# nktoan/h-edit

Measured on AMD Instinct MI355X. Metric: edited images/sec (512^2, 50 steps, K Langevin), higher is better.
Workload: dtype bf16

## Files before the change

### h-edit_amd/csrc/attn.hip

```cpp
#include "common.h"
#include "kernels.h"
#include <type_traits>

namespace {

typedef __attribute__((ext_vector_type(4))) unsigned u32x4;

__device__ __forceinline__ float fast_exp2(float x) { return __builtin_amdgcn_exp2f(x); }
#ifndef SA_BURST
#define SA_BURST 0
#endif

template <int D>
struct HeadCfg {
  static constexpr int DP = (D + 15) / 16 * 16;
  static constexpr int DK = DP / 16;
  static constexpr int DT = (D + 31) / 32;
  static constexpr int KS = DP + 8;
  static constexpr int DCH = D / 8;
};

__device__ __forceinline__ bf16x8 pack_p8(const float* p) {
  union { uint32_t u[4]; bf16x8 v; } x;
  x.u[0] = pack_bf16x2(p[0], p[1]);
// ... 547 lines not shown
    write_out(o[0], 1.0f / denom(0), q_base);
  }
}

template <int D, int QG, int NS>
int launch_self(const SelfAttnParams& p, hipStream_t st) {
  using C = SelfCfg<D, QG>;
#ifdef SA_OCC1
  constexpr int LDS = C::TOTAL > 84 * 1024 ? C::TOTAL : 84 * 1024;
#else
  constexpr int LDS = C::TOTAL;
#endif
  if (int rc = hedit_dyn_lds(reinterpret_cast<const void*>(&self_attn_kernel<D, QG, NS>), LDS)) return rc;
  dim3 grid(cdiv(p.N, 128 * QG) * p.heads * p.B);
  hipLaunchKernelGGL((self_attn_kernel<D, QG, NS>), grid, dim3(256), LDS, st, p);
  LAUNCH_CHECK();
  return HEDIT_OK;
}

constexpr int CTXP = HEDIT_CTXP;
constexpr int WS = 100;

template <int D>
struct CrossSmem {
  using H = HeadCfg<D>;
  static constexpr int K_BYTES = 96 * H::KS * 2;
  static constexpr int V_BYTES = H::DT * 32 * WS * 2;
  static constexpr int MIX_BYTES = 96 * WS * 2;
  static constexpr int BV_BYTES = 96 * 4;
  static constexpr int TOTAL = K_BYTES + V_BYTES + MIX_BYTES + BV_BYTES;
};

template <int D>
__global__ __launch_bounds__(256, (D <= 80 ? 2 : 1)) void cross_attn_kernel(CrossAttnParams p) {
  using H = HeadCfg<D>;
  using S = CrossSmem<D>;
  extern __shared__ __attribute__((aligned(16))) char smem[];
  bf16_t* sK = reinterpret_cast<bf16_t*>(smem);
  bf16_t* sV = reinterpret_cast<bf16_t*>(smem + S::K_BYTES);
  bf16_t* sM = reinterpret_cast<bf16_t*>(smem + S::K_BYTES + S::V_BYTES);
  float* sB = reinterpret_cast<float*>(smem + S::K_BYTES + S::V_BYTES + S::MIX_BYTES);

  const int tid = threadIdx.x, lane = tid & 63, wave = tid >> 6;
  const int ql = lane & 31, hi = lane >> 5;
  const int h = blockIdx.y;
  const int item = blockIdx.z;
  const bool is_pair = item < p.n_pairs;
  const int b0 = is_pair ? p.pair_src[item] : p.singles[item - p.n_pairs];
  const int b1 = is_pair ? p.pair_tar[item] : -1;
  const int q_row = blockIdx.x * 128 + wave * 32 + ql;
  const bool q_ok = q_row < p.N;

  for (int i = tid; i < (S::K_BYTES + S::V_BYTES) / 8; i += 256) reinterpret_cast<uint2*>(smem)[i] = make_uint2(0, 0);
  if (is_pair) {
    const bf16_t* src = p.mixT + (long)item * 96 * 96;
    for (int i = tid; i < 96 * 12; i += 256) {
      const int row = i / 12, c = i - row * 12;
      const uint4 u = *reinterpret_cast<const uint4*>(src + row * 96 + c * 8);
      uint2* dst = reinterpret_cast<uint2*>(sM + row * WS + c * 8);
      dst[0] = make_uint2(u.x, u.y);
      dst[1] = make_uint2(u.z, u.w);
    }
    if (tid < 96) sB[tid] = p.bvec[(long)item * 96 + tid];
  }
  __syncthreads();

  auto stage = [&](int b) {
    const bf16_t* kbase = p.k + (long)b * CTXP * p.ldk + h * D;
    for (int idx = tid; idx < CTXP * H::DCH; idx += 256) {
      const int row = idx / H::DCH, c = idx - row * H::DCH;
      *reinterpret_cast<uint4*>(sK + row * H::KS + c * 8) =
          *reinterpret_cast<const uint4*>(kbase + (long)row * p.ldk + c * 8);
    }
    const bf16_t* vbase = p.vt + (long)h * D * p.ldvt + (long)b * CTXP;
    for (int idx = tid; idx < D * (CTXP / 8); idx += 256) {
      const int row = idx / (CTXP / 8), c = idx - row * (CTXP / 8);
      const uint4 u = *reinterpret_cast<const uint4*>(vbase + (long)row * p.ldvt + c * 8);
      uint2* dst = reinterpret_cast<uint2*>(sV + row * WS + c * 8);
      dst[0] = make_uint2(u.x, u.y);
      dst[1] = make_uint2(u.z, u.w);
    }
  };

  auto load_q = [&](int b, bf16x8* qf) {
    const bf16_t* qp = p.q + ((long)b * p.N + (q_ok ? q_row : 0)) * p.ldq + h * D;
#pragma unroll
    for (int ks = 0; ks < H::DK; ++ks) {
      const int c = ks * 16 + hi * 8;
      union { uint4 u; bf16x8 v; } x;
      x.u = make_uint4(0, 0, 0, 0);
      if (q_ok && c < D) x.u = *reinterpret_cast<const uint4*>(qp + c);
      qf[ks] = x.v;
    }
  };

  auto probs = [&](const bf16x8* qf, float (*pr)[16]) {
    float mx = -1e30f;
#pragma unroll
    for (int nt = 0; nt < 3; ++nt) {
      f32x16 s;
#pragma unroll
      for (int r = 0; r < 16; ++r) s[r] = 0.f;
#pragma unroll
      for (int ks = 0; ks < H::DK; ++ks) {
        const bf16x8 kf = *reinterpret_cast<const bf16x8*>(sK + (nt * 32 + ql) * H::KS + ks * 16 + hi * 8);
        s = MFMA_32x32x16_ST(kf, qf[ks], s, 0, 0, 0);
      }
#pragma unroll
      for (int r = 0; r < 16; ++r) {
        const int n = nt * 32 + (r & 3) + 8 * (r >> 2) + 4 * hi;
        const float v = n < HEDIT_MAXW ? s[r] : -1e30f;
        pr[nt][r] = v;
        mx = fmaxf(mx, v);
      }
    }
    mx = fmaxf(mx, __shfl_xor(mx, 32, 64));
    float ls = 0.f;
// ... 73 lines not shown
    for (int r = 0; r < 16; ++r) mix[nt][r] = 0.f;
#pragma unroll
    for (int wt = 0; wt < 3; ++wt)
#pragma unroll
      for (int s2 = 0; s2 < 2; ++s2) {
        const bf16x8 mf = read_perm_frag(sM, nt * 32 + ql, WS, wt * 32 + 16 * s2 + 4 * hi);
        mix[nt] = MFMA_32x32x16_ST(mf, pf[wt][s2], mix[nt], 0, 0, 0);
      }
  }
  __syncthreads();
  stage(b1);
  __syncthreads();
  load_q(b1, qf);
  probs(qf, pr);
#pragma unroll
  for (int nt = 0; nt < 3; ++nt)
#pragma unroll
    for (int g = 0; g < 4; ++g) {
      const f32x4 bv = *reinterpret_cast<const f32x4*>(sB + nt * 32 + 8 * g + 4 * hi);
#pragma unroll
      for (int j = 0; j < 4; ++j) pr[nt][g * 4 + j] = mix[nt][g * 4 + j] + bv[j] * pr[nt][g * 4 + j];
    }
  accumulate_store(1, pr);
#pragma unroll
  for (int nt = 0; nt < 3; ++nt) { pf[nt][0] = pack_p8(pr[nt]); pf[nt][1] = pack_p8(pr[nt] + 8); }
  pv_and_write(b1, pf);
}

template <int D>
int launch_cross(const CrossAttnParams& p, hipStream_t st) {
  using S = CrossSmem<D>;
  if (int rc = hedit_dyn_lds(reinterpret_cast<const void*>(&cross_attn_kernel<D>), S::TOTAL)) return rc;
  dim3 grid(cdiv(p.N, 128), p.heads, p.n_pairs + p.n_single);
  hipLaunchKernelGGL((cross_attn_kernel<D>), grid, dim3(256), S::TOTAL, st, p);
  LAUNCH_CHECK();
  return HEDIT_OK;
}

template <bool STORE>
__global__ __launch_bounds__(256) void attn_probs_kernel(AttnProbsParams p) {
  __shared__ float qs[16][168];
  extern __shared__ float sc_rows[];
  const int bh = blockIdx.y, h = bh % p.heads;
  int b = bh / p.heads;
  if constexpr (STORE) {
    const int pair = b >> 1;
    b = (b & 1) ? p.pair_tar[pair] : p.pair_src[pair];
  }
  const int bq = (STORE && p.qk_src) ? p.qk_src[b] : b;
  const int q0 = blockIdx.x * 16, tid = threadIdx.x;
  for (int i = tid; i < 16 * p.d; i += 256) {
    const int r = i / p.d, c = i % p.d;
    const int q = q0 + r;
    qs[r][c] = q < p.N ? bf16_to_f32(p.q[((long)bq * p.N + q) * p.ldq + h * p.d + c]) : 0.f;
  }
  __syncthreads();
  float* out = STORE ? sc_rows : p.probs + ((long)bh * p.N + q0) * p.M;
  const int rows = min(16, p.N - q0);
  for (int m = tid; m < p.M; m += 256) {
    const bf16_t* kp = p.k + ((long)bq * p.kstride + m) * p.ldk + h * p.d;
    float acc[16];
#pragma unroll
    for (int r = 0; r < 16; ++r) acc[r] = 0.f;
    for (int c = 0; c < p.d; c += 8) {
      const uint4 raw = *reinterpret_cast<const uint4*>(kp + c);
      const uint32_t w[4] = {raw.x, raw.y, raw.z, raw.w};
#pragma unroll
// ... 95 lines not shown
  hipLaunchKernelGGL(attn_probs_kernel<true>, dim3(cdiv(p.N, 16), 2 * p.B * p.heads), dim3(256), lds, st, p);
  LAUNCH_CHECK();
  return HEDIT_OK;
}

int attn_apply_launch(const AttnProbsParams& p, hipStream_t st) {
  ARG_CHECK(p.d % 8 == 0 && p.d <= 160, "attn_apply: head dim must be a multiple of 8, at most 160");
  ARG_CHECK(p.M > 0 && p.N > 0 && p.M <= p.kstride, "attn_apply: extents");
  hipLaunchKernelGGL(attn_apply_kernel, dim3(cdiv(p.N, 16), p.B * p.heads), dim3(256), 0, st, p);
  LAUNCH_CHECK();
  return HEDIT_OK;
}

int self_attn_launch(const SelfAttnParams& p_in, hipStream_t st) {
  SelfAttnParams p = p_in;
  p.test_flags = hedit_test_flags();
  ARG_CHECK(p.N % 64 == 0, "self_attn: N must be a multiple of 64");
  ARG_CHECK(p.ldq % 8 == 0 && p.ldk % 8 == 0 && p.ldvt % 8 == 0 && p.ldo % 4 == 0, "self_attn: strides");
  switch (p.d) {
    case 32: return launch_self<32, 2, 2>(p, st);
    case 40: return launch_self<40, 2, 2>(p, st);
    case 64: return launch_self<64, 2, 2>(p, st);
    case 80: return launch_self<80, 1, 1>(p, st);
    case 160: return launch_self<160, 1, 1>(p, st);
    default:
      hedit_set_error("self_attn: unsupported head dim " + std::to_string(p.d) + " (32,40,64,80,160)");
      return HEDIT_ERR_ARG;
  }
}

int cross_attn_launch(const CrossAttnParams& p, hipStream_t st) {
  ARG_CHECK(p.n_pairs + p.n_single > 0, "cross_attn: nothing to do");
  ARG_CHECK(p.ldq % 8 == 0 && p.ldk % 8 == 0 && p.ldvt % 8 == 0 && p.ldo % 4 == 0, "cross_attn: strides");
  switch (p.d) {
    case 32: return launch_cross<32>(p, st);
    case 40: return launch_cross<40>(p, st);
    case 64: return launch_cross<64>(p, st);
    case 80: return launch_cross<80>(p, st);
    case 160: return launch_cross<160>(p, st);
    default:
      hedit_set_error("cross_attn: unsupported head dim " + std::to_string(p.d) + " (32,40,64,80,160)");
      return HEDIT_ERR_ARG;
  }
}
```

### h-edit_amd/csrc/c_api.hip

```cpp
#include "../../include/hedit.h"
#include <exception>
#include <map>
#include <mutex>
#include <new>
#include <set>
#include <utility>

#include "common.h"
#include "kernels.h"

static thread_local std::string g_last_error;
void hedit_set_error(const std::string& msg) { g_last_error = msg; }

int hedit_abi_catch() noexcept {
  try {
    try {
      throw;
    } catch (const std::bad_alloc&) {
      g_last_error = "out of host memory inside libhedit_hip";
    } catch (const std::exception& e) {
      g_last_error = std::string("C++ exception inside libhedit_hip: ") + e.what();
    } catch (...) {
      g_last_error = "unknown C++ exception inside libhedit_hip";
    }
// ... 196 lines not shown
  p.bias = bias_packed;
  p.C = reinterpret_cast<bf16_t*>(C);
  p.ldc = ldc;
  p.geglu = 1;
  return gemm_launch(p, 1, nullptr, S(stream));
} catch (...) { return hedit_abi_catch(); }

int hedit_k_ffn_channels(void) { return ffn_fused_channels(); }
size_t hedit_k_ffn_stream_bytes(int with_outer_layers) { return ffn_stream_bytes(with_outer_layers, with_outer_layers); }
size_t hedit_k_ffn_bias_bytes(void) { return ffn_bias_bytes(); }

int hedit_k_ffn_pack(const float* w1, const float* b1, const float* w2, const float* w_pre, const float* w_post, void* stream_out,
                     float* bias1_out, void* stream) try {
  ARG_CHECK(w1 && b1 && w2 && stream_out && bias1_out && ((w_pre == nullptr) == (w_post == nullptr)), "ffn_pack args");
  const int outer = w_pre != nullptr;
  bf16_t* so = reinterpret_cast<bf16_t*>(stream_out);
  int rc = ffn_pack_launch(w1, 1, outer, outer, so, S(stream));
  if (rc == HEDIT_OK) rc = ffn_pack_launch(w2, 2, outer, outer, so, S(stream));
  if (rc == HEDIT_OK && outer) rc = ffn_pack_launch(w_pre, 0, 1, 1, so, S(stream));
  if (rc == HEDIT_OK && outer) rc = ffn_pack_launch(w_post, 3, 1, 1, so, S(stream));
  if (rc != HEDIT_OK) return rc;
  return ffn_pack_bias_launch(b1, bias1_out, S(stream));
} catch (...) { return hedit_abi_catch(); }

int hedit_k_ffn_fused(const void* x, int64_t ldx, const float* gamma, const float* beta, float eps, const void* w_stream,
                      const float* bias1_packed, const float* bias2, void* out, int64_t ldo, int M, int C, void* stream) try {
  FfnParams f{};
  f.x = reinterpret_cast<const bf16_t*>(x); f.ldx = (long)ldx; f.gamma = gamma; f.beta = beta; f.eps = eps;
  f.stream = reinterpret_cast<const bf16_t*>(w_stream); f.bias1p = bias1_packed; f.bias2 = bias2;
  f.out = reinterpret_cast<bf16_t*>(out); f.ldo = (long)ldo; f.M = M; f.C = C;
  return ffn_fused_launch(f, S(stream));
} catch (...) { return hedit_abi_catch(); }

int hedit_k_ffn_chain(const void* a, int64_t lda, const void* t1, int64_t ldt1, const void* x, int64_t ldx, const float* bias_pre,
                      const float* gamma, const float* beta, float eps, const void* w_stream, const float* bias1_packed, const float* bias2,
                      const float* bias_post, void* out, int64_t ldo, int M, int C, void* stream) try {
  ARG_CHECK(a && t1 && x, "ffn_chain args");
  FfnParams f{};
  f.a = reinterpret_cast<const bf16_t*>(a); f.lda = (long)lda;
  f.x = reinterpret_cast<const bf16_t*>(t1); f.ldx = (long)ldt1;
  f.r2 = reinterpret_cast<const bf16_t*>(x); f.ldr2 = (long)ldx;
  f.bias_pre = bias_pre; f.bias_post = bias_post;
  f.gamma = gamma; f.beta = beta; f.eps = eps;
  f.stream = reinterpret_cast<const bf16_t*>(w_stream); f.bias1p = bias1_packed; f.bias2 = bias2;
  f.out = reinterpret_cast<bf16_t*>(out); f.ldo = (long)ldo; f.M = M; f.C = C;
  return ffn_fused_launch(f, S(stream));
} catch (...) { return hedit_abi_catch(); }

size_t hedit_k_lin_chain_stream_bytes(int n_out) { return lin_chain_stream_bytes(n_out == 3 ? 4 : 2); }

int hedit_k_lin_chain_pack(const float* w_pre, const float* w0, const float* w1, const float* w2, float scale0, void* stream_out,
                           void* stream) try {
  ARG_CHECK(w_pre && w0 && stream_out && ((w1 == nullptr) == (w2 == nullptr)), "lin_chain_pack args");
  const int layers = w1 ? 4 : 2;
  bf16_t* so = reinterpret_cast<bf16_t*>(stream_out);
  int rc = lin_chain_pack_launch(w_pre, 0, 1.f, layers, so, S(stream));
  if (rc == HEDIT_OK) rc = lin_chain_pack_launch(w0, 1, scale0, layers, so, S(stream));
  if (rc == HEDIT_OK && w1) rc = lin_chain_pack_launch(w1, 2, 1.f, layers, so, S(stream));
  if (rc == HEDIT_OK && w1) rc = lin_chain_pack_launch(w2, 3, 1.f, layers, so, S(stream));
  return rc;
} catch (...) { return hedit_abi_catch(); }

int hedit_k_lin_chain(const void* a, int64_t lda, const void* r1, int64_t ldr1, const float* gn_ss, int rows_per_image,
                      const float* bias_pre, const float* gamma, const float* beta, float eps, const void* w_stream, void* out_mid,
                      int64_t ldmid, void* out_q, int64_t ldq, void* out_k, int64_t ldk, void* out, int64_t ldo, int M, int C,
                      void* stream) try {
  LinChainParams c{};
  c.a = reinterpret_cast<const bf16_t*>(a); c.lda = (long)lda; c.r1 = reinterpret_cast<const bf16_t*>(r1); c.ldr1 = (long)ldr1;
  c.bias_pre = bias_pre; c.gamma = gamma; c.beta = beta; c.eps = eps; c.stream = reinterpret_cast<const bf16_t*>(w_stream);
  c.out_mid = reinterpret_cast<bf16_t*>(out_mid); c.ldmid = (long)ldmid; c.out = reinterpret_cast<bf16_t*>(out); c.ldo = (long)ldo;
  c.M = M; c.C = C; c.gn_ss = gn_ss; c.rows_per_image = rows_per_image;
  c.out_q = reinterpret_cast<bf16_t*>(out_q); c.ldq = (long)ldq; c.out_k = reinterpret_cast<bf16_t*>(out_k); c.ldk = (long)ldk;
  return lin_chain_launch(c, S(stream));
} catch (...) { return hedit_abi_catch(); }

int hedit_storage_is_f16(void) { return HEDIT_F16; }

int hedit_test_set_flags(int flags) try {
  ARG_CHECK(flags >= 0 && flags <= 15, "hedit_test_set_flags: bit 0 drained ring waits, bit 1 exact self-attention pass, bit 2 pixel-UNet GroupNorm statistics path flipped, bit 3 no persistent linear kernel");
  g_test_flags.store(flags, std::memory_order_relaxed);
  return HEDIT_OK;
} catch (...) { return hedit_abi_catch(); }

int hedit_k_lin_chain_sched(const void* a, int64_t lda, const void* r1, int64_t ldr1, const float* gn_ss, int rows_per_image,
                            const float* bias_pre, const float* gamma, const float* beta, float eps, const void* w_stream, void* out_mid,
                            int64_t ldmid, void* out_q, int64_t ldq, void* out_k, int64_t ldk, void* out, int64_t ldo, int M, int C,
                            int sched, void* stream) try {
  LinChainParams c{};
  c.a = reinterpret_cast<const bf16_t*>(a); c.lda = (long)lda; c.r1 = reinterpret_cast<const bf16_t*>(r1); c.ldr1 = (long)ldr1;
  c.bias_pre = bias_pre; c.gamma = gamma; c.beta = beta; c.eps = eps; c.stream = reinterpret_cast<const bf16_t*>(w_stream);
  c.out_mid = reinterpret_cast<bf16_t*>(out_mid); c.ldmid = (long)ldmid; c.out = reinterpret_cast<bf16_t*>(out); c.ldo = (long)ldo;
  c.M = M; c.C = C; c.gn_ss = gn_ss; c.rows_per_image = rows_per_image;
  c.out_q = reinterpret_cast<bf16_t*>(out_q); c.ldq = (long)ldq; c.out_k = reinterpret_cast<bf16_t*>(out_k); c.ldk = (long)ldk;
  return lin_chain_launch_sched(c, sched, S(stream));
} catch (...) { return hedit_abi_catch(); }

size_t hedit_k_groupnorm_ws_bytes(int B, int HW, int C) { return groupnorm_ws_bytes(B, HW, C); }

int hedit_k_groupnorm_affine(const void* x, const float* gamma, const float* beta, int B, int HW, int C, int G, float eps, void* ws,
                             float* ss_out, void* stream) try {
  ARG_CHECK(x && gamma && beta && ws && ss_out, "groupnorm_affine args");
  const float* ss = nullptr;
  int rc = groupnorm_affine_launch(reinterpret_cast<const bf16_t*>(x), gamma, beta, B, HW, C, G, eps, reinterpret_cast<float*>(ws), S(stream), &ss);
  if (rc != HEDIT_OK) return rc;
  HIP_TRY(hipMemcpyAsync(ss_out, ss, (size_t)B * C * 2 * sizeof(float), hipMemcpyDeviceToDevice, S(stream)));
  return HEDIT_OK;
} catch (...) { return hedit_abi_catch(); }

int hedit_k_groupnorm(const void* x, void* y, const float* gamma, const float* beta, int B, int HW, int C, int G,
                      float eps, int silu, void* ws, void* stream) try {
  ARG_CHECK(x && y && gamma && beta && ws, "groupnorm args");
  return groupnorm_launch(reinterpret_cast<const bf16_t*>(x), reinterpret_cast<bf16_t*>(y), gamma, beta, B, HW, C, G,
// ... 132 lines not shown
```

### h-edit_amd/csrc/ffn.hip

```cpp
#include <type_traits>
#include <utility>

#include "common.h"
#include "kernels.h"

namespace {

typedef __attribute__((ext_vector_type(4))) unsigned u32x4;
typedef __attribute__((ext_vector_type(2))) unsigned u32x2;

constexpr int FC = 320;
constexpr int FKS = FC / 16;
constexpr int FNB = FC / 32;
constexpr int FH = 4 * FC;
constexpr int FPAIRS = FH / 16;
constexpr int UNIT = 10240;
constexpr int ITER_BYTES = 3 * UNIT;
constexpr int BANKS = 5, AHEAD = 4;
constexpr int NITER = FPAIRS + 2;
constexpr int LIN_ITERS = 7;
constexpr int LIN_FRAGS = FKS * FNB;
__host__ __device__ constexpr int stream_iters(bool pre, bool post) { return (pre ? LIN_ITERS : 0) + NITER + (post ? LIN_ITERS : 0) + AHEAD; }
constexpr int BIAS_OFF = BANKS * ITER_BYTES;
constexpr int BIAS_BYTES = FPAIRS * 128;
// ... 51 lines not shown
      }
    } else if (t - 2 >= 0 && t - 2 < FPAIRS) {
      owner = 2;
      if (which == 2) {
#pragma unroll
        for (int e = 0; e < 8; ++e) v[e] = w[(long)((j - 20) * 32 + row) * FH + (t - 2) * 16 + ffn_unit_of_reg(e, hi)];
      }
    }
  }
  if (which != owner) return;
  uint4 o = pack8(v);
  *reinterpret_cast<uint4*>(reinterpret_cast<char*>(stream) + idx * 16) = o;
}

__global__ __launch_bounds__(256) void ffn_pack_bias_kernel(const float* __restrict__ b1, float* __restrict__ out) {
  const int idx = blockIdx.x * 256 + threadIdx.x;
  if (idx >= BIAS_BYTES / 4) return;
  const int t = idx >> 5, hi = (idx >> 4) & 1, r = idx & 15;
  out[idx] = r < 8 ? b1[t * 16 + ffn_unit_of_reg(r, hi)] : b1[FH + t * 16 + ffn_unit_of_reg(r - 8, hi)];
}

struct ChainKernelParams {
  const bf16_t* a; long lda;
  const bf16_t* r1; long ldr1;
  const bf16_t* r2; long ldr2;
  const float* bias_pre;
  const float* gamma; const float* beta; float eps;
  const bf16_t* stream;
  const float* bias1p;
  const float* bias2;
  const float* bias_post;
  bf16_t* out; long ldo;
  int M;
};

template <class F, int... I>
__device__ __forceinline__ void static_for_impl(F&& f, std::integer_sequence<int, I...>) {
  (f(std::integral_constant<int, I>{}), ...);
}
template <int N, class F>
__device__ __forceinline__ void static_for(F&& f) {
  static_for_impl(f, std::make_integer_sequence<int, N>{});
}

__device__ __forceinline__ void mfma_s(f32x16& acc, const bf16x8& w, const bf16x8& a) {
  asm volatile("v_mfma_f32_32x32x16_" MFMA_ST_SFX " %0, %1, %2, %0" : "+v"(acc) : "v"(w), "a"(a));
}
__device__ __forceinline__ void mfma_s0(f32x16& acc, const bf16x8& w, const bf16x8& a, const f32x16& c) {
  asm volatile("v_mfma_f32_32x32x16_" MFMA_ST_SFX " %0, %1, %2, %3" : "=&v"(acc) : "v"(w), "a"(a), "v"(c));
}
__device__ __forceinline__ void mfma_z(f32x16& acc, const bf16x8& w, const bf16x8& a) {
  asm volatile("v_mfma_f32_32x32x16_" MFMA_ST_SFX " %0, %1, %2, 0" : "=&v"(acc) : "v"(w), "a"(a));
}
__device__ __forceinline__ void mfma_o(f32x16& acc, const bf16x8& w, const bf16x8& h) {
  asm volatile("v_mfma_f32_32x32x16_" MFMA_ST_SFX " %0, %1, %2, %0" : "+a"(acc) : "v"(w), "v"(h));
}
__device__ __forceinline__ void mfma_l(f32x16& acc, const bf16x8& w, const bf16x8& a) {
  asm volatile("v_mfma_f32_32x32x16_" MFMA_ST_SFX " %0, %1, %2, %0" : "+a"(acc) : "v"(w), "a"(a));
}

struct Gelu8 {
  float x[8], q[8], g[8];
  uint32_t h[4];
};
constexpr int GELU_OPS = 15 * 8 + 4;
#define GELU_PIN(v) asm volatile("" : "+v"(v))
// ... 10 lines not shown
      else if constexpr (st == 4) g.q[e] = __builtin_fmaf(g.q[e], __builtin_fabsf(x), 5.21099924e-02f);
      else if constexpr (st == 5) g.q[e] = __builtin_fmaf(g.q[e], __builtin_fabsf(x), 1.04427174e+00f);
      else if constexpr (st <= 9) g.q[e] = g.q[e] * g.q[e];
      else g.q[e] = __builtin_amdgcn_rcpf(g.q[e]);
      GELU_PIN(g.q[e]);
    } else {
      if constexpr (st == 11) g.g[e] = __builtin_fmaxf(g.x[e], 0.f);
      else if constexpr (st == 12) g.g[e] = __builtin_fmaf(-__builtin_fabsf(g.x[e]), g.q[e], g.g[e]);
      else if constexpr (st == 13) { g.q[e] = Se[e] + So[e]; GELU_PIN(g.q[e]); }
      else g.g[e] = g.g[e] * g.q[e];
      GELU_PIN(g.g[e]);
    }
  } else {
    constexpr int p = K - 120;
    g.h[p] = pack_bf16x2(g.g[2 * p], g.g[2 * p + 1]);
    GELU_PIN(g.h[p]);
  }
}
template <int LO, int HI>
__device__ __forceinline__ void gelu_ops(Gelu8& g, const f32x16& Se, const f32x16& So) {
  static_for<HI - LO>([&](auto k) { gelu_op<LO + decltype(k)::value>(g, Se, So); });
}

template <bool PRE, bool POST, bool DRAIN = false>
__global__ __launch_bounds__(256, 1) void ffn_chain_kernel(ChainKernelParams p) {
  extern __shared__ __attribute__((aligned(16))) char smem[];
  const int tid = threadIdx.x;
  const int lane = tid & 63;
  const int wave = __builtin_amdgcn_readfirstlane(tid >> 6);
  const int lm = lane & 31, hi = lane >> 5;
  const int m_wave = blockIdx.x * BLOCK_ROWS + wave * ROWS_PER_WAVE;
  int row_c = m_wave + lm;
  if (row_c > p.M - 1) row_c = p.M - 1;

#if defined(__HIP_DEVICE_COMPILE__)
  const __amdgpu_buffer_rsrc_t rs_w = __builtin_amdgcn_make_buffer_rsrc(const_cast<bf16_t*>(p.stream), (short)0, (int)(stream_iters(PRE, POST) * ITER_BYTES), 0x00020000);
  const __amdgpu_buffer_rsrc_t rs_b = __builtin_amdgcn_make_buffer_rsrc(const_cast<float*>(p.bias1p), (short)0, (int)BIAS_BYTES, 0x00020000);
#endif
  unsigned dma_voff[2];
  dma_voff[0] = (unsigned)(wave * 1024 + lane * 16);
  dma_voff[1] = (unsigned)((wave + 28 > 29 ? 29 : wave + 28) * 1024 + lane * 16);
  const int dma_last = (wave + 28 > 29 ? 29 : wave + 28) * 1024;
  auto dma_piece = [&](int it, int bank, int k) __attribute__((always_inline)) {
#if defined(__HIP_DEVICE_COMPILE__)
    if (k < 7)
      __builtin_amdgcn_raw_ptr_buffer_load_lds(rs_w, (__attribute__((address_space(3))) void*)(smem + bank * ITER_BYTES + wave * 1024 + k * 4096), 16,
                                               dma_voff[0], it * ITER_BYTES + k * 4096, 0, 0);
    else
      __builtin_amdgcn_raw_ptr_buffer_load_lds(rs_w, (__attribute__((address_space(3))) void*)(smem + bank * ITER_BYTES + dma_last), 16, dma_voff[1],
                                               it * ITER_BYTES, 0, 0);
#else
    (void)it; (void)bank; (void)k;
#endif
  };

#if defined(__HIP_DEVICE_COMPILE__)
  for (int i = wave; i < BIAS_BYTES / 1024; i += 4)
    __builtin_amdgcn_raw_ptr_buffer_load_lds(rs_b, (__attribute__((address_space(3))) void*)(smem + BIAS_OFF + i * 1024), 16,
                                             (unsigned)(i * 1024 + lane * 16), 0, 0, 0);
#endif
#pragma unroll
  for (int it = 0; it < AHEAD; ++it)
#pragma unroll
    for (int k = 0; k < PPW; ++k) dma_piece(it, it, k);

  f32x16 O[FNB];
  auto load_rows = [&](const bf16_t* src, long ld, const float* bias) __attribute__((always_inline)) {
    const bf16_t* rp = src + (long)row_c * ld + hi * 8;
    u32x4 raw[FKS];
#pragma unroll
    for (int k = 0; k < FKS; ++k) raw[k] = *reinterpret_cast<const u32x4*>(rp + k * 16);
#pragma unroll
    for (int k = 0; k < FKS; ++k) {
      const auto s0 = __builtin_amdgcn_permlane32_swap(raw[k][0], raw[k][2], false, false);
      const auto s1 = __builtin_amdgcn_permlane32_swap(raw[k][1], raw[k][3], false, false);
      const unsigned half[2][2] = {{s0[0], s1[0]}, {s0[1], s1[1]}};
#pragma unroll
      for (int c2 = 0; c2 < 2; ++c2) {
        const int c = 2 * k + c2, nb = c / 4, q = c % 4;
        f32x4 bb = {0.f, 0.f, 0.f, 0.f};
        if (bias) bb = *reinterpret_cast<const f32x4*>(bias + nb * 32 + q * 8 + hi * 4);
        O[nb][4 * q] = st_lo(half[c2][0]) + bb[0];
        O[nb][4 * q + 1] = st_hi(half[c2][0]) + bb[1];
        O[nb][4 * q + 2] = st_lo(half[c2][1]) + bb[2];
        O[nb][4 * q + 3] = st_hi(half[c2][1]) + bb[3];
      }
    }
  };
  auto settle = [&]() __attribute__((always_inline)) {
    asm volatile("s_nop 7\n\ts_nop 7\n\ts_nop 7\n\ts_nop 7\n\ts_nop 7\n\ts_nop 7\n\ts_nop 7\n\ts_nop 7" ::: "memory");
#pragma unroll
    for (int nb = 0; nb < FNB; ++nb) asm volatile("" : "+a"(O[nb]));
  };
  auto publish = [&]() __attribute__((always_inline)) {
#pragma unroll
    for (int nb = 0; nb < FNB; ++nb) asm volatile("" : "+a"(O[nb]));
    asm volatile("s_nop 3" ::: "memory");
  };

  bf16x8 Xn[FKS];
  load_rows(p.r1, p.ldr1, PRE ? p.bias_pre : nullptr);
  if constexpr (PRE) {
    const bf16_t* src = p.a + (long)row_c * p.lda + hi * 8;
#pragma unroll
    for (int ks = 0; ks < FKS; ++ks) {
      const u32x4 raw = *reinterpret_cast<const u32x4*>(src + ks * 16);
      Xn[ks] = __builtin_bit_cast(bf16x8, raw);
      asm volatile("" : "+a"(Xn[ks]));
    }
  }
  auto frags_from_acc = [&](auto ln_c, float mean, float rstd) __attribute__((always_inline)) {
    constexpr bool LN = decltype(ln_c)::value;
#pragma unroll
    for (int ks = 0; ks < FKS; ++ks) {
      float o[8];
#pragma unroll
      for (int h2 = 0; h2 < 2; ++h2) {
        const int q = 2 * (ks % 2) + h2;
        f32x4 gg = {1.f, 1.f, 1.f, 1.f}, bb = {0.f, 0.f, 0.f, 0.f};
        if constexpr (LN) {
          gg = *reinterpret_cast<const f32x4*>(p.gamma + (ks / 2) * 32 + q * 8 + hi * 4);
          bb = *reinterpret_cast<const f32x4*>(p.beta + (ks / 2) * 32 + q * 8 + hi * 4);
        }
#pragma unroll
        for (int j = 0; j < 4; ++j) {
          const float v = O[ks / 2][4 * q + j];
          o[4 * h2 + j] = LN ? (v - mean) * rstd * gg[j] + bb[j] : v;
        }
      }
      const u32x4 pk = {pack_bf16x2(o[0], o[1]), pack_bf16x2(o[2], o[3]), pack_bf16x2(o[4], o[5]), pack_bf16x2(o[6], o[7])};
      Xn[ks] = __builtin_bit_cast(bf16x8, pk);
      asm volatile("" : "+a"(Xn[ks]));
    }
  };
// ... 144 lines not shown
      if constexpr (F1 && b >= 10 && b < 14) {
        constexpr int q = b - 10;
        const f32x4 v = *reinterpret_cast<const f32x4*>(smem + (bias_rd + q * 16));
        bnext[4 * q] = v[0]; bnext[4 * q + 1] = v[1]; bnext[4 * q + 2] = v[2]; bnext[4 * q + 3] = v[3];
      }
      if constexpr (b % 3 == 1 && b / 3 < PPW) dma_piece(it + AHEAD, pbank, b / 3);
      if constexpr (GELU) gelu_ops<(b * GELU_OPS) / NB, ((b + 1) * GELU_OPS) / NB>(G, Sprev, Sprev2);
      __builtin_amdgcn_sched_barrier(0);
    });
    boundary();
    if constexpr (GELU) {
      Hgelu = (u32x4){G.h[0], G.h[1], G.h[2], G.h[3]};
      asm volatile("" : "+v"(Hgelu));
    }
    if constexpr (F1) {
      binit = bnext;
      ++pair;
      if (pair + 1 < FPAIRS) bias_rd += 128;
    }
    advance(nbank, nbase);
  };
  using T = std::true_type;
  using F = std::false_type;
  for (int tt = 0; tt < FPAIRS / 2; ++tt) {
    ff_iteration(T{}, T{}, T{}, Sa, Sa2, Sb, Sb2, Hb, Ha);
    ff_iteration(T{}, T{}, T{}, Sb, Sb2, Sa, Sa2, Ha, Hb);
  }
  ff_iteration(F{}, T{}, T{}, Sa, Sa2, Sb, Sb2, Hb, Ha);
  ff_iteration(F{}, F{}, F{}, Sb, Sb2, Sa, Sa2, Ha, Hb);

  if constexpr (POST) {
    settle();
    frags_from_acc(std::false_type{}, 0.f, 1.f);
    load_rows(p.r2, p.ldr2, p.bias_post);
    publish();
    asm volatile("s_waitcnt vmcnt(0)" ::: "memory");
#pragma unroll
    for (int j = 0; j < LEAD; ++j) pre[j] = rd(frag_rd, false, j);
    linear_layer(std::false_type{});
  }

  settle();
  asm volatile("s_waitcnt vmcnt(0) lgkmcnt(0)\n\ts_barrier" ::: "memory");
  constexpr int PITCH = FC * 2 + 16;
  constexpr int STAGE = 24576;
  static_assert(ROWS_PER_WAVE * PITCH <= STAGE && 4 * STAGE <= BIAS_OFF, "epilogue staging must fit the ring");
  char* stage = smem + wave * STAGE;
#pragma unroll
  for (int nb = 0; nb < FNB; ++nb) {
#pragma unroll
    for (int q = 0; q < 4; ++q) {
      u32x2 o;
      o[0] = pack_bf16x2(O[nb][4 * q], O[nb][4 * q + 1]);
      o[1] = pack_bf16x2(O[nb][4 * q + 2], O[nb][4 * q + 3]);
      *reinterpret_cast<u32x2*>(stage + lm * PITCH + (nb * 32 + q * 8 + hi * 4) * 2) = o;
    }
  }
  asm volatile("s_waitcnt lgkmcnt(0)" ::: "memory");
  constexpr int CPR = FC / 8;
  constexpr int ITER = ROWS_PER_WAVE * CPR / 64;
  static_assert(ROWS_PER_WAVE * CPR % 64 == 0, "rows must divide evenly over the lanes");
  u32x4 ov[ITER];
#pragma unroll
  for (int i = 0; i < ITER; ++i) {
    const int idx = lane + i * 64;
    const int rl = idx / CPR, c = idx - rl * CPR;
    ov[i] = *reinterpret_cast<const u32x4*>(stage + rl * PITCH + c * 16);
// ... 18 lines not shown
  ARG_CHECK((which != 0 || pre) && (which != 3 || post), "ffn_pack: this stream has no such layer");
  const long total = (long)stream_iters(pre != 0, post != 0) * (ITER_BYTES / 16);
  hipLaunchKernelGGL(ffn_pack_kernel, dim3(cdiv(total, 256)), dim3(256), 0, st, w, which, pre, post, stream);
  LAUNCH_CHECK();
  return HEDIT_OK;
}

int ffn_pack_bias_launch(const float* b1, float* out, hipStream_t st) {
  hipLaunchKernelGGL(ffn_pack_bias_kernel, dim3(cdiv(BIAS_BYTES / 4, 256)), dim3(256), 0, st, b1, out);
  LAUNCH_CHECK();
  return HEDIT_OK;
}

template <bool PRE, bool POST>
static int launch_chain(const ChainKernelParams& k, hipStream_t st) {
  if (hedit_test_drained()) {
    if (int rc = hedit_dyn_lds(reinterpret_cast<const void*>(&ffn_chain_kernel<PRE, POST, true>), LDS_TOTAL)) return rc;
    hipLaunchKernelGGL((ffn_chain_kernel<PRE, POST, true>), dim3(cdiv(k.M, BLOCK_ROWS)), dim3(256), LDS_TOTAL, st, k);
    LAUNCH_CHECK();
    return HEDIT_OK;
  }
  if (int rc = hedit_dyn_lds(reinterpret_cast<const void*>(&ffn_chain_kernel<PRE, POST>), LDS_TOTAL)) return rc;
  hipLaunchKernelGGL((ffn_chain_kernel<PRE, POST>), dim3(cdiv(k.M, BLOCK_ROWS)), dim3(256), LDS_TOTAL, st, k);
  LAUNCH_CHECK();
  return HEDIT_OK;
}

int ffn_fused_launch(const FfnParams& f, hipStream_t st) {
  ARG_CHECK(f.C == FC, "ffn: the fused feed-forward exists for C = 320");
  ARG_CHECK(f.M > 0 && f.ldx % 8 == 0 && f.ldo % 8 == 0, "ffn: rows must be 16-byte aligned");
  ARG_CHECK(f.x && f.out && f.stream && f.bias1p && f.bias2 && f.gamma && f.beta, "ffn: null");
  const bool pre = f.a != nullptr, post = f.r2 != nullptr;
  ARG_CHECK(pre == post, "ffn: the chain exists with both outer linear layers or with neither");
  ChainKernelParams k{};
  k.r1 = f.x; k.ldr1 = f.ldx; k.gamma = f.gamma; k.beta = f.beta; k.eps = f.eps;
  k.stream = f.stream; k.bias1p = f.bias1p; k.bias2 = f.bias2; k.out = f.out; k.ldo = f.ldo; k.M = f.M;
  if (pre) {
    ARG_CHECK(f.lda % 8 == 0 && f.ldr2 % 4 == 0 && f.ldx % 4 == 0 && f.bias_pre && f.bias_post, "ffn chain: alignment / biases");
    k.a = f.a; k.lda = f.lda; k.r2 = f.r2; k.ldr2 = f.ldr2; k.bias_pre = f.bias_pre; k.bias_post = f.bias_post;
    return launch_chain<true, true>(k, st);
  }
  return launch_chain<false, false>(k, st);
}
```

### h-edit_amd/csrc/kernels.h

```cpp
#pragma once
#include "common.h"

struct GemmParams {
  const bf16_t* A;
  const bf16_t* W;
  int M, N, K;
  int lda;
  int mode;
  int Hin, Win, Cin, Hout, Wout;
  const float* bias;
  const bf16_t* residual;
  int ldr;
  bf16_t* C;
  int ldc;
  float* partial;
  int splits, kt_per_split;
  int n_fastest;
  const bf16_t* zeros;
  unsigned a_bytes, w_bytes;
  int geglu;
  int asym;
  float* raw_f32;
  int chunk_kt;
  const float *ln_gamma, *ln_beta;
  bf16_t* ln_out;
  float ln_eps;
  int* ln_done;
  float* gn_part;
  int op_bf16;
};
#ifndef GEMM_NOMINAL_BATCH
#define GEMM_NOMINAL_BATCH 4
#endif
int gemm_prepare();
int gemm_pick_bn(int N);
int gemm_pick_splits(int M, int N, int K, int force);
int gemm_canonical_chunk(int M_nom, int N_nom, int K);
int gemm_plan_splits(int M, int N, int K, int chunk_kt);
size_t gemm_partial_bytes(int M, int N, int splits);
int gemm_launch(GemmParams p, int splits, float* partial_ws, hipStream_t st);
bool pgemm_supported(const GemmParams& p, int splits, int bn);
int pgemm_launch(const GemmParams& p, int bn, hipStream_t st);
bool pconv_supported(const GemmParams& p, int splits, int bn);
int pconv_launch(const GemmParams& p, int bn, hipStream_t st);

struct FfnParams {
  const bf16_t* x; long ldx;
  const float* gamma; const float* beta; float eps;
  const bf16_t* stream;
  const float* bias1p;
  const float* bias2;
  bf16_t* out; long ldo;
  int M, C;
  const bf16_t* a; long lda;
  const bf16_t* r2; long ldr2;
  const float* bias_pre; const float* bias_post;
};
struct LinChainParams {
  const bf16_t* a; long lda;
  const bf16_t* r1; long ldr1;
  const float* bias_pre;
  const float* gamma; const float* beta; float eps;
  const bf16_t* stream;
  bf16_t* out_mid; long ldmid;
  bf16_t* out; long ldo;
  int M, C;
  const float* gn_ss; int rows_per_image;
  bf16_t* out_q; long ldq; bf16_t* out_k; long ldk;
};
int lin_chain_launch(const LinChainParams& c, hipStream_t st);
int lin_chain_launch_sched(const LinChainParams& c, int sched, hipStream_t st);
size_t lin_chain_stream_bytes(int layers);
int lin_chain_pack_launch(const float* w, int layer, float scale, int layers, bf16_t* stream, hipStream_t st);
int ffn_fused_channels();
size_t ffn_stream_bytes(int pre, int post);
size_t ffn_bias_bytes();
int ffn_pack_launch(const float* w, int which, int pre, int post, bf16_t* stream, hipStream_t st);
int ffn_pack_bias_launch(const float* b1, float* out, hipStream_t st);
int ffn_fused_launch(const FfnParams& f, hipStream_t st);

#define HEDIT_MAXW 77
#define HEDIT_WPAD 96
#define HEDIT_CTXP 80

size_t groupnorm_ws_bytes(int B, int HW, int C);
int groupnorm_launch(const bf16_t* x, bf16_t* y, const float* gamma, const float* beta, int B,
                     int HW, int C, int G, float eps, int silu, float* ws, hipStream_t st,
                     float* stats = nullptr);
bool groupnorm_from_parts_supported(int HW, int C, int G);
size_t groupnorm_from_parts_ws_bytes(int B);
int groupnorm_from_parts_launch(const bf16_t* x, bf16_t* y, const float* gamma, const float* beta, int B, int HW, int C, int G,
                                float eps, int silu, const float* part_a, int ca, const float* part_b, int cb, float* ws,
                                hipStream_t st);
int groupnorm_affine_launch(const bf16_t* x, const float* gamma, const float* beta, int B, int HW, int C, int G, float eps,
                            float* ws, hipStream_t st, const float** ss_out);
int layernorm_launch(const bf16_t* x, bf16_t* y, const float* gamma, const float* beta, long rows,
                     int C, float eps, hipStream_t st);
bool splitk_reduce_ln_supported(int C);
int splitk_reduce_ln_launch(const float* partial, int splits, const float* bias, const bf16_t* residual, int ldr, bf16_t* out,
                            bf16_t* y, const float* gamma, const float* beta, long rows, int C, float eps, hipStream_t st);
int geglu_launch(const bf16_t* x, bf16_t* y, long rows, int inner, hipStream_t st);
#define HEDIT_ROWMAP_MAX 512
struct RowMap { uint16_t src[HEDIT_ROWMAP_MAX]; };
int concat_launch(const bf16_t* a, int ca, const bf16_t* b, int cb, bf16_t* y, long rows, hipStream_t st,
                  const RowMap* b_map = nullptr, int rows_per_image = 0);
int gather_rows_launch(const void* const* src, void* const* dst, int n, int B, long row_bytes, const RowMap& map, hipStream_t st);
int f32_to_bf16_launch(const float* x, bf16_t* y, long n, hipStream_t st);
int ctx_pad_launch(const float* x, bf16_t* y, int B, int dim, hipStream_t st);
int gemv_launch(const bf16_t* W, const float* x, const float* b0, const float* b1, float* out,
                int N, int K, int silu, hipStream_t st);
int copy_rows_launch(bf16_t* x, const int* src, int B, long row_elems, hipStream_t st);
int timestep_embed_launch(float t, float* out, int dim, hipStream_t st);
int timestep_embed_ddpm_launch(float t, float* out, int dim, hipStream_t st);
int conv_in_launch(const float* x, const float* w, const float* bias, bf16_t* y, int B, int Cin,
                   int H, int W, int Cout, hipStream_t st);
int conv_out_launch(const bf16_t* x, const bf16_t* w, const float* bias, float* y, int B, int H,
                    int W, int C, int Cout, hipStream_t st);
int rows_to_nchw_launch(const float* src, const float* bias, float* dst, int B, long HW, int ld, int Cout, hipStream_t st);
int softmax_rows_launch(const float* s, bf16_t* p, long rows, int N, float scale, hipStream_t st);
int softmax_blockdiag_launch(const float* s, bf16_t* p, long rows, int T, int ld, float scale, hipStream_t st);
int mix1x1_nchw_launch(const float* x, const float* w, const float* bias, float* y, int B, int Cin, int Cout, long HW,
                       float pre_scale, hipStream_t st);
int quant_mean_launch(const bf16_t* h, const float* w, const float* bias, float* y, int B, long HW, int Cm, int Cout, hipStream_t st);
int pack_linear_launch(const float* w, bf16_t* out, long n, float scale, hipStream_t st);
int pack_conv3x3_launch(const float* w_oihw, bf16_t* out, int O, int I, hipStream_t st);
int pack_geglu_rows_launch(const float* w, bf16_t* out_bf16, float* out_f32, int rows, int K, hipStream_t st);

size_t groupnorm_bwd_ws_bytes(int B, int HW, int C);
int groupnorm_bwd_launch(const bf16_t* x, const bf16_t* dy, const bf16_t* add, bf16_t* dx, const float* gamma,
                         const float* beta, const float* stats, int B, int HW, int C, int G, int silu, float* ws,
                         hipStream_t st);
int softmax_bwd_launch(const bf16_t* p, const float* dp, bf16_t* ds, long rows, int N, float scale, hipStream_t st);
int transpose_bf16_launch(const bf16_t* src, bf16_t* dst, int R, int C, hipStream_t st);
int sum2x2_launch(const bf16_t* du, bf16_t* dx, int B, int H, int W, int C, hipStream_t st);
int pack_conv3x3_dgrad_launch(const float* w_oihw, bf16_t* out, int O, int I, hipStream_t st);
int pack_linear_t_launch(const float* w, bf16_t* out, int O, int I, hipStream_t st);
int flip_oihw_launch(const float* w, float* out, int O, int I, int k, hipStream_t st);

struct SelfAttnParams {
  const bf16_t* q; int ldq;
  const bf16_t* k; int ldk;
  const bf16_t* vt; long ldvt;
  bf16_t* out; int ldo;
  int B, N, heads, d;
  const int* qk_src;
  const int* kv_src;
  int test_flags;
};
int self_attn_launch(const SelfAttnParams& p, hipStream_t st);

struct CrossAttnParams {
  const bf16_t* q; int ldq;
  const bf16_t* k; int ldk;
  const bf16_t* vt; long ldvt;
  bf16_t* out; int ldo;
  int B, N, heads, d;
  int n_pairs;
  const int* pair_src;
  const int* pair_tar;
  const bf16_t* mixT;
  const float* bvec;
  float* store;
  const int* singles;
  int n_single;
};
int cross_attn_launch(const CrossAttnParams& p, hipStream_t st);

struct AttnProbsParams {
  const bf16_t* q; int ldq;
  const bf16_t* k; int ldk;
  const bf16_t* vt; long ldvt;
  float* probs;
  bf16_t* out; int ldo;
  int B, N, M, kstride, heads, d;
  const int *pair_src, *pair_tar, *qk_src;
};
int attn_probs_launch(const AttnProbsParams& p, hipStream_t st);
int attn_self_store_launch(const AttnProbsParams& p, hipStream_t st);
int attn_apply_launch(const AttnProbsParams& p, hipStream_t st);

struct StepCoef {
  float sqrt_ab_t, sqrt_1m_ab_t;
  float sqrt_ab_prev;
  float dir_coef;
  float noise_coef;
  float w_src, w_hat, w_tar;
  float coeff;
  float w_rec;
};
int step_base_launch(const float* eps, const float* xt, const float* z, float* x_prev, int n_img,
                     int elems, int eps_rows_per_img, StepCoef c, hipStream_t st);
int step_pair_launch(const float* e_u, const float* e_c, const float* xt, const float* z, float* x_next, int n_img, int elems,
                     int n_kinds, const StepCoef* c, hipStream_t st);
int step_invert_launch(const float* e_u, const float* e_c, const float* xt, float* x_prev, float* z_out, int n_img,
                       int elems, StepCoef c, hipStream_t st);
int step_update_launch(const float* e_u_src, const float* e_c_src, const float* e_u_tar,
                       const float* e_c_tar, long stride_img, const float* x_k, const float* x_base,
// ... 56 lines not shown
```

### h-edit_amd/csrc/unet.hip

```cpp
#include <array>
#include <map>
#include <string>
#include <vector>

#include "../../include/hedit.h"
#include "common.h"
#include "exec.h"
#include "kernels.h"

#define TRY(expr)                        \
  do {                                   \
    int _rc = (expr);                    \
    if (_rc != HEDIT_OK) return _rc;     \
  } while (0)

namespace {

struct Slot {
  std::string name;
  int kind;
  void* dst;
  size_t numel;
  int O, I;
  float scale;
  bool loaded;
  int ndim;
  int dims[4];
  int which = 0, lay = 0;
};

struct Res {
  int cin, cout, temb_off;
  float *n1g, *n1b, *n2g, *n2b, *conv2_b, *sc_b;
// ... 13 lines not shown
  std::vector<Res> res;
  std::vector<Attn> attn;
  bool has_attn = false, has_sampler = false;
  bf16_t* samp_w = nullptr;
  float* samp_b = nullptr;
  int ch = 0;
};

}

struct hedit_unet {
  hedit_unet_cfg cfg;
  std::vector<void*> owned;
  std::vector<Slot> slots;
  std::map<std::string, int> index;
  int temb_dim = 0, temb_total = 0;
  float *conv_in_w = nullptr, *conv_in_b = nullptr, *te1_b = nullptr, *te2_b = nullptr;
  bf16_t *te1_w = nullptr, *te2_w = nullptr, *temb_w_all = nullptr, *conv_out_w = nullptr;
  float *temb_b_all = nullptr, *conv1_b_all = nullptr, *gn_out_g = nullptr, *gn_out_b = nullptr, *conv_out_b = nullptr;
  std::vector<Block> down, up;
  Res mid_res[2];
  Attn mid_attn;
  int32_t* iota = nullptr;
  int iota_cap = 0;
  bool prof_on = false;
  std::vector<hipEvent_t> prof_pool;
  struct ProfRec { int kind; double flops, bytes; int e0, e1; int m = 0, n = 0, k = 0, tag = 0; };
  std::vector<ProfRec> prof_recs;
  size_t prof_next = 0;
  hedit_attn_hook_fn hook = nullptr;
  void* hook_user = nullptr;
  bf16_t *wk2_all = nullptr, *wv2_all = nullptr;
  int ctx_n = 0, ctx_next = 0;
  std::map<std::array<int, 4>, size_t> ws_cache;
};

namespace {

template <class T>
T* dalloc(hedit_unet* h, size_t n) {
  void* p = nullptr;
  if (hipMalloc(&p, n * sizeof(T) > 0 ? n * sizeof(T) : 16) != hipSuccess) return nullptr;
  h->owned.push_back(p);
  return reinterpret_cast<T*>(p);
}

void add_slot(hedit_unet* h, const std::string& name, int kind, void* dst, size_t numel, int O = 0, int I = 0, float scale = 1.f) {
  Slot s{name, kind, dst, numel, O, I, scale, false, 1, {(int)numel, 1, 1, 1}};
  if (kind == 1) { s.ndim = 2; s.dims[0] = O; s.dims[1] = I; }
  if (kind == 2) { s.ndim = 4; s.dims[0] = O; s.dims[1] = I; s.dims[2] = 3; s.dims[3] = 3; }
  if (kind == 1 && (name.find("proj_in.weight") != std::string::npos || name.find("proj_out.weight") != std::string::npos ||
                    name.find("conv_shortcut.weight") != std::string::npos)) {
    s.ndim = 4; s.dims[2] = 1; s.dims[3] = 1;
  }
  h->index[name] = (int)h->slots.size();
  h->slots.push_back(s);
}
float* f32p(hedit_unet* h, const std::string& name, size_t n, float* dst = nullptr) {
  if (!dst) dst = dalloc<float>(h, n);
  add_slot(h, name, 0, dst, n);
  return dst;
}
bf16_t* linp(hedit_unet* h, const std::string& name, int O, int I, bf16_t* dst = nullptr, float scale = 1.f) {
  if (!dst) dst = dalloc<bf16_t>(h, (size_t)O * I);
  add_slot(h, name, 1, dst, (size_t)O * I, O, I, scale);
  return dst;
}
// ... 79 lines not shown
    a.w_o2 = linp(h, tb + ".attn2.to_out.0.weight", C, C);
  }
  a.o2_b = f32p(h, tb + ".attn2.to_out.0.bias", C);
  a.ln3g = f32p(h, tb + ".norm3.weight", C);
  a.ln3b = f32p(h, tb + ".norm3.bias", C);
  if (chain) {
    stream_slot(tb + ".ff.net.0.proj.weight", a.ffs, 0, 1, 8 * C, C, 1.f, 2);
    add_slot(h, tb + ".ff.net.0.proj.bias", 6, a.ff1_bp, (size_t)8 * C);
    stream_slot(tb + ".ff.net.2.weight", a.ffs, 0, 2, C, 4 * C, 1.f, 2);
  } else {
    a.ff1 = linp(h, tb + ".ff.net.0.proj.weight", 8 * C, C);
    h->slots.back().kind = 3;
    a.ff1_b = f32p(h, tb + ".ff.net.0.proj.bias", 8 * C);
    h->slots.back().kind = 4;
    a.ff2 = linp(h, tb + ".ff.net.2.weight", C, 4 * C);
  }
  a.ff2_b = f32p(h, tb + ".ff.net.2.bias", C);
  if (chain) {
    stream_slot(pre + ".proj_out.weight", a.ffs, 0, 3, C, C, 1.f, 4);
  } else {
    a.pout = linp(h, pre + ".proj_out.weight", C, C);
  }
  a.pout_b = f32p(h, pre + ".proj_out.bias", C);
  return a;
}

struct Fwd {
  hedit_unet* h;
  int B;
  hipStream_t st;
  Arena ar;
  const hedit_p2p_plan* plan;
  const float* temb_all;
  const bf16_t* ctxb;
  const bf16_t* k2_all = nullptr;
  const bf16_t* vt2_all = nullptr;
  int store_idx = 0;
  int store_self_idx = 0;
  int tblock = 0;
  int rblock = 0;
  int place = 0;
  int hook_layer = 0;
  const RowMap* map = nullptr;
  bool dry() const { return ar.dry; }
};

struct BatchScope {
  Fwd& f;
  int saved;
  BatchScope(Fwd& f_, int rows) : f(f_), saved(f_.B) { f.B = rows; }
  ~BatchScope() { f.B = saved; }
  BatchScope(const BatchScope&) = delete;
  BatchScope& operator=(const BatchScope&) = delete;
};

#define RUN(f, expr)            \
  do {                          \
    if (!(f).dry()) TRY(expr);  \
  } while (0)

enum { PK_CONV = 0, PK_LINEAR = 1, PK_SELF_ATTN = 2, PK_CROSS_ATTN = 3, PK_NORM = 4, PK_OTHER = 5, PK_COUNT = 6 };

struct ProfScope {
  hedit_unet* h;
  hipStream_t st;
  int rec = -1;
  ProfScope(Fwd& f, int kind, double flops, double bytes = 0.0);
// ... 215 lines not shown
        ap.B = pl->n_pairs; ap.N = N; ap.M = N; ap.kstride = N; ap.heads = heads; ap.d = d;
        ap.pair_src = pl->pair_src; ap.pair_tar = pl->pair_tar; ap.qk_src = sp.qk_src;
        RUN(f, attn_self_store_launch(ap, f.st));
      }
      f.store_self_idx++;
    }
  }
  f.ar.free(qk);
  f.ar.free(vt);
  TRY(aalloc(f, &t1, M * C));
  TRY(aalloc(f, &q2, M * C));
  if (chain) {
    LinChainParams lc{};
    lc.a = ao; lc.lda = C; lc.r1 = t0; lc.ldr1 = C; lc.bias_pre = a.o1_b;
    lc.gamma = a.ln2g; lc.beta = a.ln2b; lc.eps = 1e-5f; lc.stream = a.k1s;
    lc.out_mid = t1; lc.ldmid = C; lc.out = q2; lc.ldo = C; lc.M = (int)M; lc.C = C;
    ProfScope ps(f, PK_LINEAR, 2.0 * M * 2.0 * C * C, 8.0 * M * C + 4.0 * C * C);
    chain_prof(f, ps, M, C, 2, 130);
    RUN(f, lin_chain_launch(lc, f.st));
  } else {
    TRY(aalloc(f, &tn, M * C));
    TRY(linear_ln(f, ao, (int)M, C, a.w_o1, C, a.o1_b, t0, t1, a.ln2g, a.ln2b, 1e-5f, tn));
    TRY(linear(f, tn, (int)M, C, a.w_q2, C, nullptr, nullptr, q2, C));
    f.ar.free(tn);
  }
  f.ar.free(ao);
  f.ar.free(t0);
  *t1_out = t1;
  *q2_out = q2;
  return HEDIT_OK;
}

int transformer_rest(Fwd& f, const Attn& a, const bf16_t* x, bf16_t* t1, bf16_t* q2, int H, int W, bf16_t** out,
                     bf16_t* dst = nullptr, int ldd = 0) {
  const int C = a.C, N = H * W, B = f.B, heads = f.h->cfg.heads, d = C / heads;
  const size_t M = (size_t)B * N;
  const hedit_p2p_plan* pl = (f.plan && f.plan->mode > 0) ? f.plan : nullptr;
  bf16_t *tn, *ao, *k2, *vt2, *t2, *gf, *t3, *y;
  const bool chain = a.ffs != nullptr;
  const int MC = B * HEDIT_CTXP;
  k2 = const_cast<bf16_t*>(f.k2_all) + a.ctx_off;
  vt2 = const_cast<bf16_t*>(f.vt2_all) + (size_t)a.ctx_off * MC;
  const int ldk2 = f.h->ctx_n;
  TRY(aalloc(f, &ao, M * C));
  {
    CrossAttnParams cp{};
    cp.q = q2; cp.ldq = C; cp.k = k2; cp.ldk = ldk2; cp.vt = vt2; cp.ldvt = MC; cp.out = ao; cp.ldo = C;
    cp.B = B; cp.N = N; cp.heads = heads; cp.d = d;
    const bool stored_layer = N <= 1024;
    if (pl) {
      cp.n_pairs = pl->n_pairs; cp.pair_src = pl->pair_src; cp.pair_tar = pl->pair_tar;
      cp.mixT = reinterpret_cast<const bf16_t*>(pl->mixT); cp.bvec = pl->bvec;
      cp.singles = pl->singles; cp.n_single = pl->n_single;
      cp.store = (pl->mode == 2 && stored_layer && pl->h_store && f.store_idx < pl->n_store) ? pl->h_store[f.store_idx] : nullptr;
    } else {
      cp.n_pairs = 0; cp.singles = f.h->iota; cp.n_single = B;
    }
    if (stored_layer) f.store_idx++;
    if (f.h->hook) {
      TRY(hooked_attention(f, cp.q, cp.ldq, cp.k, cp.ldk, cp.vt, cp.ldvt, ao, C, N, HEDIT_MAXW, HEDIT_CTXP, heads, d, 1));
    } else {
      ProfScope ps(f, PK_CROSS_ATTN, 4.0 * B * (double)N * HEDIT_MAXW * C, 4.0 * M * C + 4.0 * MC * C);
      RUN(f, cross_attn_launch(cp, f.st));
    }
  }
  f.ar.free(q2);
  if (chain) {
    if (dst) {
      y = dst;
    } else {
      TRY(aalloc(f, &y, M * C));
    }
    FfnParams fp{};
    fp.a = ao; fp.lda = C; fp.x = t1; fp.ldx = C; fp.r2 = x; fp.ldr2 = C;
    fp.bias_pre = a.o2_b; fp.bias_post = a.pout_b;
    fp.gamma = a.ln3g; fp.beta = a.ln3b; fp.eps = 1e-5f;
    fp.stream = a.ffs; fp.bias1p = a.ff1_bp; fp.bias2 = a.ff2_b; fp.out = y; fp.ldo = dst ? ldd : C; fp.M = (int)M; fp.C = C;
    {
      ProfScope ps(f, PK_LINEAR, 2.0 * M * 14.0 * C * C, 8.0 * M * C + 28.0 * C * C);
      chain_prof(f, ps, M, C, 14, 128);
      RUN(f, ffn_fused_launch(fp, f.st));
    }
    f.ar.free(ao);
    f.ar.free(t1);
    *out = y;
    return HEDIT_OK;
  }
  TRY(aalloc(f, &t2, M * C));
  TRY(aalloc(f, &tn, M * C));
  TRY(linear_ln(f, ao, (int)M, C, a.w_o2, C, a.o2_b, t1, t2, a.ln3g, a.ln3b, 1e-5f, tn));
  f.ar.free(ao);
  f.ar.free(t1);
  TRY(aalloc(f, &gf, M * 4 * C));
  {
    GemmParams gp{};
    gp.A = tn; gp.W = a.ff1; gp.M = (int)M; gp.N = 8 * C; gp.K = C; gp.lda = C; gp.mode = 0;
    gp.bias = a.ff1_b; gp.residual = nullptr; gp.ldr = 0; gp.C = gf; gp.ldc = 4 * C; gp.geglu = 1;
    ProfScope ps(f, PK_LINEAR, 2.0 * gp.M * gp.N * gp.K, gemm_alg_bytes(f, gp));
    RUN(f, gemm_launch(gp, 1, nullptr, f.st));
  }
  f.ar.free(tn);
  TRY(aalloc(f, &t3, M * C));
  TRY(linear(f, gf, (int)M, 4 * C, a.ff2, C, a.ff2_b, t2, t3, C));
  f.ar.free(gf);
  f.ar.free(t2);

  if (dst) {
    y = dst;
  } else {
    TRY(aalloc(f, &y, M * C));
  }
  TRY(linear(f, t3, (int)M, C, a.pout, C, a.pout_b, x, y, dst ? ldd : C));
  f.ar.free(t3);
  *out = y;
  return HEDIT_OK;
}

int transformer(Fwd& f, const Attn& a, const bf16_t* x, int H, int W, bf16_t** out, bf16_t* dst = nullptr, int ldd = 0) {
  bf16_t *t1, *q2;
  TRY(transformer_stem(f, a, x, H, W, &t1, &q2));
  return transformer_rest(f, a, x, t1, q2, H, W, out, dst, ldd);
}

struct Skip { bf16_t* p; int C; bool per_latent = false; };

bool stem_shareable(const hedit_unet* h, const hedit_p2p_plan* plan, int D, int B, int N0) {
  if (D >= B || h->hook || h->down.empty() || !h->down[0].has_attn) return false;
  const hedit_p2p_plan* pl = (plan && plan->mode > 0) ? plan : nullptr;
  if (!pl) return true;
  if (pl->feat_src && pl->feat_resblock <= 0) return false;
  if (pl->kv_src && pl->kv_first_block <= 0) return false;
  if (pl->qk_src && N0 <= (pl->qk_max_tokens > 0 ? pl->qk_max_tokens : 1024) && pl->qk_first_block <= 0) return false;
  if (pl->mode == 2 && pl->h_store_self && pl->n_store_self > 0 && N0 <= 1024) return false;
  return true;
}

int broadcast_stem(Fwd& f, size_t row_elems, bf16_t** x, bf16_t** t1, bf16_t** q2, int D) {
  bf16_t** narrow[3] = {x, t1, q2};
  bf16_t* wide[3];
  const void* src[3];
  void* dst[3];
  for (int i = 0; i < 3; ++i) {
    TRY(aalloc(f, &wide[i], (size_t)f.B * row_elems));
    src[i] = *narrow[i];
    dst[i] = wide[i];
  }
  {
    ProfScope ps(f, PK_OTHER, 0.0, 3.0 * (D + f.B) * (double)row_elems * sizeof(bf16_t));
    RUN(f, gather_rows_launch(src, dst, 3, f.B, (long)(row_elems * sizeof(bf16_t)), *f.map, f.st));
  }
  for (int i = 0; i < 3; ++i) {
    f.ar.free(*narrow[i]);
    *narrow[i] = wide[i];
  }
  return HEDIT_OK;
}

int forward_impl(hedit_unet* h, const float* x, float t, const float* ctx, int B, int H0, int W0,
                 const hedit_p2p_plan* plan, float* eps_out, void* ws, size_t ws_bytes, hipStream_t st,
                 bool dry, size_t* peak, int D = 0, const RowMap* map = nullptr) {
  const hedit_unet_cfg& c = h->cfg;
  Fwd f;
  f.h = h; f.B = B; f.st = st; f.plan = plan; f.map = map;
  f.ar.base = reinterpret_cast<char*>(ws); f.ar.cap = ws_bytes; f.ar.dry = dry;
  const int ch0 = c.block_out_channels[0];

  if (!dry && h->iota_cap < B) {
    hedit_set_error("batch larger than " + std::to_string(h->iota_cap) + " rows");
    return HEDIT_ERR_ARG;
  }

  bf16_t* ctxb;
  TRY(aalloc(f, &ctxb, (size_t)B * HEDIT_CTXP * c.cross_attention_dim));
  RUN(f, ctx_pad_launch(ctx, ctxb, B, c.cross_attention_dim, st));
  f.ctxb = ctxb;
  {
    const int MC = B * HEDIT_CTXP;
    bf16_t *k2a, *vt2a;
    TRY(aalloc(f, &k2a, (size_t)MC * h->ctx_n));
    TRY(aalloc(f, &vt2a, (size_t)MC * h->ctx_n));
    TRY(linear(f, ctxb, MC, c.cross_attention_dim, h->wk2_all, h->ctx_n, nullptr, nullptr, k2a, h->ctx_n));
    TRY(linear(f, h->wv2_all, h->ctx_n, c.cross_attention_dim, ctxb, MC, nullptr, nullptr, vt2a, MC, 2));
    f.k2_all = k2a;
    f.vt2_all = vt2a;
  }

  float *te0, *te1, *te2, *temb_all;
  TRY(aalloc(f, &te0, (size_t)ch0));
  TRY(aalloc(f, &te1, (size_t)h->temb_dim));
  TRY(aalloc(f, &te2, (size_t)h->temb_dim));
  TRY(aalloc(f, &temb_all, (size_t)h->temb_total));
  RUN(f, timestep_embed_launch(t, te0, ch0, st));
  RUN(f, gemv_launch(h->te1_w, te0, h->te1_b, nullptr, te1, h->temb_dim, ch0, 0, st));
  RUN(f, gemv_launch(h->te2_w, te1, h->te2_b, nullptr, te2, h->temb_dim, h->temb_dim, 1, st));
  RUN(f, gemv_launch(h->temb_w_all, te2, h->temb_b_all, h->conv1_b_all, temb_all, h->temb_total, h->temb_dim, 1, st));
  f.temb_all = temb_all;

  int H = H0, W = W0;
  const bool share = D > 0 && stem_shareable(h, plan, D, B, H0 * W0);
  float* xrows = nullptr;
  if (D > 0 && !share) {
    const size_t img = (size_t)c.in_channels * H * W;
    TRY(aalloc(f, &xrows, (size_t)B * img));
    const void* src[1] = {x};
    void* dst[1] = {xrows};
    ProfScope ps(f, PK_OTHER, 0.0, (double)(D + B) * img * sizeof(float));
    RUN(f, gather_rows_launch(src, dst, 1, B, (long)(img * sizeof(float)), *map, st));
    x = xrows;
  }
  bf16_t* cur;
  {
    BatchScope rows(f, share ? D : B);
    TRY(aalloc(f, &cur, (size_t)f.B * H * W * ch0));
    RUN(f, conv_in_launch(x, h->conv_in_w, h->conv_in_b, cur, f.B, c.in_channels, H, W, ch0, st));
  }
  if (xrows) f.ar.free(xrows);
  std::vector<Skip> skips;
  skips.push_back({cur, ch0, share});

  for (int i = 0; i < c.n_levels; ++i) {
    Block& blk = h->down[i];
    for (size_t j = 0; j < blk.res.size(); ++j) {
      const bool stem = share && i == 0 && j == 0;
      bf16_t *y, *t1 = nullptr, *q2 = nullptr;
      {
        BatchScope rows(f, stem ? D : B);
        TRY(resblock(f, blk.res[j], cur, H, W, &y));
        if (blk.has_attn) {
          f.place = 0;
          TRY(transformer_stem(f, blk.attn[j], y, H, W, &t1, &q2));
        }
      }
      cur = y;
      if (stem) TRY(broadcast_stem(f, (size_t)H * W * blk.ch, &cur, &t1, &q2, D));
      if (blk.has_attn) {
        bf16_t* z;
        TRY(transformer_rest(f, blk.attn[j], cur, t1, q2, H, W, &z));
        f.ar.free(cur);
        cur = z;
      }
      skips.push_back({cur, blk.ch});
    }
    if (blk.has_sampler) {
      bf16_t* y;
      TRY(aalloc(f, &y, (size_t)B * (H / 2) * (W / 2) * blk.ch));
      TRY(conv3x3(f, cur, H, W, blk.ch, blk.samp_w, blk.ch, blk.samp_b, nullptr, y, 2));
      H /= 2; W /= 2;
      cur = y;
      skips.push_back({cur, blk.ch});
    }
  }

  {
    bf16_t *y, *z, *w;
    TRY(resblock(f, h->mid_res[0], cur, H, W, &y));
    f.place = 1;
    TRY(transformer(f, h->mid_attn, y, H, W, &z));
    f.ar.free(y);
    TRY(resblock(f, h->mid_res[1], z, H, W, &w));
    f.ar.free(z);
    cur = w;
  }
  int cur_c = c.block_out_channels[c.n_levels - 1];

  bool in_cat = false;
  bf16_t* cat_next = nullptr;
  for (int i = 0; i < c.n_levels; ++i) {
    Block& blk = h->up[i];
    for (size_t j = 0; j < blk.res.size(); ++j) {
      Skip s = skips.back();
// ... 45 lines not shown
      H *= 2; W *= 2;
      cur = dst;
      in_cat = true;
      cat_next = dst;
    }
  }

  {
    bf16_t* a;
    TRY(aalloc(f, &a, (size_t)B * H * W * ch0));
    TRY(groupnorm(f, cur, a, h->gn_out_g, h->gn_out_b, H * W, ch0, 1e-5f, 1));
    if (c.out_channels != 4 || ch0 % 64 != 0) {
      RUN(f, conv_out_launch(a, h->conv_out_w, h->conv_out_b, eps_out, B, H, W, ch0, c.out_channels, st));
    } else {
      float* prod;
      const size_t M = (size_t)B * H * W;
      TRY(aalloc(f, &prod, M * 4));
      GemmParams p{};
      p.mode = 1; p.Hin = H; p.Win = W; p.Cin = ch0; p.Hout = H; p.Wout = W;
      p.A = a; p.W = h->conv_out_w; p.M = (int)M; p.N = 4; p.K = 9 * ch0; p.lda = ch0; p.raw_f32 = prod; p.ldc = 4;
      TRY(run_gemm(f, p));
      RUN(f, rows_to_nchw_launch(prod, h->conv_out_b, eps_out, B, (long)H * W, 4, 4, st));
      f.ar.free(prod);
    }
    f.ar.free(a);
    f.ar.free(cur);
  }
  if (peak) *peak = f.ar.peak;
  return HEDIT_OK;
}

}

extern "C" {

int hedit_unet_create(const hedit_unet_cfg* cfg, hedit_unet** out) try {
  ARG_CHECK(cfg && out, "null");
  ARG_CHECK(cfg->n_levels >= 2 && cfg->n_levels <= HEDIT_MAX_LEVELS, "n_levels");
  ARG_CHECK(cfg->in_channels <= 8 && cfg->out_channels <= 4, "in/out channels");
  ARG_CHECK(cfg->cross_attention_dim % 64 == 0, "cross_attention_dim % 64");
  for (int i = 0; i < cfg->n_levels; ++i) {
    ARG_CHECK(cfg->block_out_channels[i] % 64 == 0, "block_out_channels % 64");
    ARG_CHECK(cfg->block_out_channels[i] % cfg->norm_num_groups == 0, "channels % groups");
    const int d = cfg->block_out_channels[i] / cfg->heads;
    ARG_CHECK(d == 32 || d == 40 || d == 64 || d == 80 || d == 160, "head dim must be one of 32,40,64,80,160");
  }
  TRY(gemm_prepare());
  hedit_unet* h = new hedit_unet();
  h->cfg = *cfg;
  const int* ch = cfg->block_out_channels;
  const int L = cfg->layers_per_block, n = cfg->n_levels;
  h->temb_dim = ch[0] * 4;

  int total = 0;
  {
    int outc = ch[0];
    for (int i = 0; i < n; ++i) { outc = ch[i]; total += L * outc; }
    total += 2 * ch[n - 1];
    for (int i = 0; i < n; ++i) total += (L + 1) * ch[n - 1 - i];
  }
  h->temb_total = total;
  h->temb_w_all = dalloc<bf16_t>(h, (size_t)total * h->temb_dim);
  h->temb_b_all = dalloc<float>(h, total);
  h->conv1_b_all = dalloc<float>(h, total);

  h->conv_in_w = f32p(h, "conv_in.weight", (size_t)ch[0] * cfg->in_channels * 9);
// ... 118 lines not shown
} catch (...) { (void)hedit_abi_catch(); return 0; }

int hedit_unet_load(hedit_unet* h, const char* name, const float* w, size_t numel, void* stream) try {
  ARG_CHECK(h && name && w, "null");
  auto it = h->index.find(name);
  if (it == h->index.end()) {
    hedit_set_error(std::string("unknown parameter: ") + name);
    return HEDIT_ERR_ARG;
  }
  Slot& s = h->slots[it->second];
  if (s.numel != numel) {
    hedit_set_error(std::string("size mismatch for ") + name + ": expected " + std::to_string(s.numel) + ", got " + std::to_string(numel));
    return HEDIT_ERR_ARG;
  }
  hipStream_t st = reinterpret_cast<hipStream_t>(stream);
  if (s.kind == 0) {
    HIP_TRY(hipMemcpyAsync(s.dst, w, numel * sizeof(float), hipMemcpyDeviceToDevice, st));
  } else if (s.kind == 1) {
    TRY(pack_linear_launch(w, reinterpret_cast<bf16_t*>(s.dst), (long)numel, s.scale, st));
  } else if (s.kind == 3) {
    TRY(pack_geglu_rows_launch(w, reinterpret_cast<bf16_t*>(s.dst), nullptr, s.O, s.I, st));
  } else if (s.kind == 4) {
    TRY(pack_geglu_rows_launch(w, nullptr, reinterpret_cast<float*>(s.dst), (int)numel, 1, st));
  } else if (s.kind == 5) {
    TRY(ffn_pack_launch(w, s.which, 1, 1, reinterpret_cast<bf16_t*>(s.dst), st));
  } else if (s.kind == 6) {
    TRY(ffn_pack_bias_launch(w, reinterpret_cast<float*>(s.dst), st));
  } else if (s.kind == 7) {
    TRY(lin_chain_pack_launch(w, s.which, s.scale, s.lay, reinterpret_cast<bf16_t*>(s.dst), st));
  } else {
    TRY(pack_conv3x3_launch(w, reinterpret_cast<bf16_t*>(s.dst), s.O, s.I, st));
  }
  s.loaded = true;
  return HEDIT_OK;
} catch (...) { return hedit_abi_catch(); }

int hedit_unet_missing(const hedit_unet* h) try {
  if (!h) return -1;
  int m = 0;
  for (auto& s : h->slots) m += s.loaded ? 0 : 1;
  return m;
} catch (...) { return hedit_abi_catch(); }

size_t hedit_unet_workspace_bytes(hedit_unet* h, int B, int height, int width) try {
  if (!h) return 0;
  const std::array<int, 4> key{B, height, width, h->hook ? 1 : 0};
  auto it = h->ws_cache.find(key);
  if (it != h->ws_cache.end()) return it->second;
  size_t need = 0;
  for (int D = 0; D <= (B <= HEDIT_ROWMAP_MAX ? B : 0); ++D) {
    size_t peak = 0;
    if (forward_impl(h, nullptr, 0.f, nullptr, B, height, width, nullptr, nullptr, nullptr, 0, nullptr, true, &peak, D) != HEDIT_OK) return 0;
    if (peak > need) need = peak;
  }
  need += 4096;
  h->ws_cache[key] = need;
  return need;
} catch (...) { (void)hedit_abi_catch(); return 0; }

static int forward_checks(hedit_unet* h, const float* x, const float* ctx, int B, int height, int width, const hedit_p2p_plan* plan,
                          float* eps_out, void* workspace) {
  ARG_CHECK(h && x && ctx && eps_out && workspace, "null");
  ARG_CHECK(B >= 1, "B");
  const int div = 1 << (h->cfg.n_levels - 1);
  ARG_CHECK(height % div == 0 && width % div == 0, "latent size must be divisible by 2^(levels-1)");
  const int lowest = (height / div) * (width / div);
  ARG_CHECK(lowest % 64 == 0, "lowest-resolution level must have a multiple of 64 tokens");
  if (hedit_unet_missing(h) != 0) {
    hedit_set_error("UNet has " + std::to_string(hedit_unet_missing(h)) + " unloaded parameters");
    return HEDIT_ERR_STATE;
  }
  ARG_CHECK(!(h->hook && plan && plan->mode > 0), "an attention hook excludes the in-kernel edits of a plan (pass plan = NULL)");
  if (plan && plan->mode > 0) {
    ARG_CHECK(plan->n_pairs >= 0 && plan->n_pairs + plan->n_single > 0, "plan rows");
    ARG_CHECK(plan->n_pairs == 0 || (plan->pair_src && plan->pair_tar && plan->mixT && plan->bvec), "plan tables");
  }
  return HEDIT_OK;
}

int hedit_unet_forward(hedit_unet* h, const float* x, float t, const float* ctx, int B, int height, int width,
                       const hedit_p2p_plan* plan, float* eps_out, void* workspace, size_t workspace_bytes,
                       void* stream) try {
  TRY(forward_checks(h, x, ctx, B, height, width, plan, eps_out, workspace));
  return forward_impl(h, x, t, ctx, B, height, width, plan, eps_out, workspace, workspace_bytes,
                      reinterpret_cast<hipStream_t>(stream), false, nullptr);
} catch (...) { return hedit_abi_catch(); }

int hedit_unet_forward_shared(hedit_unet* h, const float* x, int D, const int* row_latent, float t, const float* ctx, int B,
                              int height, int width, const hedit_p2p_plan* plan, float* eps_out, void* workspace,
                              size_t workspace_bytes, void* stream) try {
  TRY(forward_checks(h, x, ctx, B, height, width, plan, eps_out, workspace));
  ARG_CHECK(row_latent && D >= 1 && D <= 65535, "row map");
  if (B > HEDIT_ROWMAP_MAX) {
    hedit_set_error("batch larger than " + std::to_string(HEDIT_ROWMAP_MAX) + " rows (the row map of shared latents)");
    return HEDIT_ERR_ARG;
  }
  ARG_CHECK(reinterpret_cast<uintptr_t>(x) % 16 == 0, "x must be 16-byte aligned");
  RowMap map{};
  for (int r = 0; r < B; ++r) {
    ARG_CHECK(row_latent[r] >= 0 && row_latent[r] < D, "row_latent entries must lie in [0, D)");
    map.src[r] = (uint16_t)row_latent[r];
  }
  return forward_impl(h, x, t, ctx, B, height, width, plan, eps_out, workspace, workspace_bytes,
                      reinterpret_cast<hipStream_t>(stream), false, nullptr, D, &map);
} catch (...) { return hedit_abi_catch(); }

int hedit_prof_enable(hedit_unet* h, int on, int max_records) try {
  ARG_CHECK(h, "null");
  if (on && (int)h->prof_pool.size() < 2 * max_records) {
    const size_t want = (size_t)2 * max_records;
    while (h->prof_pool.size() < want) {
      hipEvent_t e;
      HIP_TRY(hipEventCreate(&e));
      h->prof_pool.push_back(e);
    }
  }
  h->prof_on = on != 0;
  return HEDIT_OK;
} catch (...) { return hedit_abi_catch(); }

int hedit_prof_reset(hedit_unet* h) try {
  ARG_CHECK(h, "null");
  h->prof_recs.clear();
  h->prof_next = 0;
  return HEDIT_OK;
} catch (...) { return hedit_abi_catch(); }

int hedit_prof_collect(hedit_unet* h, int kind, double* total_ms, double* total_flops, int64_t* count) try {
  ARG_CHECK(h && total_ms && total_flops && count && kind >= 0 && kind < PK_COUNT, "prof args");
  double ms = 0, fl = 0;
  int64_t n = 0;
  for (auto& r : h->prof_recs) {
    if (r.kind != kind) continue;
    float t = 0.f;
    HIP_TRY(hipEventElapsedTime(&t, h->prof_pool[r.e0], h->prof_pool[r.e1]));
    ms += t;
    fl += r.flops;
// ... 74 lines not shown
```

### h-edit_amd/hedit/_lib.py

```python
import ctypes as C
import os

_HERE = os.path.dirname(os.path.abspath(__file__))
STORAGE = os.environ.get("HEDIT_STORAGE", "bf16").lower()
if STORAGE not in ("bf16", "f16"):
    raise ValueError(f"HEDIT_STORAGE must be bf16 or f16, not {STORAGE!r}")
LIB_PATH = os.path.join(_HERE, "libhedit_hip_f16.so" if STORAGE == "f16" else "libhedit_hip.so")
HEDIT_MAX_LEVELS = 8


class UnetCfg(C.Structure):
    _fields_ = [("in_channels", C.c_int), ("out_channels", C.c_int), ("sample_size", C.c_int),
                ("n_levels", C.c_int),
                ("block_out_channels", C.c_int * HEDIT_MAX_LEVELS),
                ("down_has_attn", C.c_int * HEDIT_MAX_LEVELS),
                ("up_has_attn", C.c_int * HEDIT_MAX_LEVELS),
                ("layers_per_block", C.c_int), ("cross_attention_dim", C.c_int),
                ("heads", C.c_int), ("norm_num_groups", C.c_int)]


class VaeCfg(C.Structure):
    _fields_ = [("in_channels", C.c_int), ("latent_channels", C.c_int), ("n_levels", C.c_int),
                ("block_out_channels", C.c_int * 4), ("layers_per_block", C.c_int),
                ("norm_num_groups", C.c_int)]


class DdpmCfg(C.Structure):
    _fields_ = [("in_channels", C.c_int), ("out_ch", C.c_int), ("ch", C.c_int), ("n_levels", C.c_int),
                ("ch_mult", C.c_int * 8), ("attn_level", C.c_int * 8), ("num_res_blocks", C.c_int),
                ("image_size", C.c_int)]


class VitCfg(C.Structure):
    _fields_ = [(n, C.c_int) for n in ("width", "layers", "heads", "patch_size", "input_resolution")]


class TextCfg(C.Structure):
    _fields_ = [(n, C.c_int) for n in ("width", "layers", "heads", "vocab_size", "context_length", "proj_dim")]


class ClipImgCfg(C.Structure):
    _fields_ = [(n, C.c_int) for n in ("width", "layers", "heads", "patch_size", "input_resolution", "embed_dim")]


class P2PPlan(C.Structure):
    _fields_ = [("mode", C.c_int), ("n_pairs", C.c_int),
                ("pair_src", C.c_void_p), ("pair_tar", C.c_void_p),
                ("singles", C.c_void_p), ("n_single", C.c_int),
                ("qk_src", C.c_void_p), ("mixT", C.c_void_p), ("bvec", C.c_void_p),
                ("h_store", C.POINTER(C.c_void_p)), ("n_store", C.c_int),
                ("kv_src", C.c_void_p), ("kv_first_block", C.c_int),
                ("qk_first_block", C.c_int), ("qk_max_tokens", C.c_int), ("feat_src", C.c_void_p), ("feat_resblock", C.c_int),
                ("h_store_self", C.POINTER(C.c_void_p)), ("n_store_self", C.c_int)]


class StepCoef(C.Structure):
    _fields_ = [(n, C.c_float) for n in ("sqrt_ab_t", "sqrt_1m_ab_t", "sqrt_ab_prev", "dir_coef",
                                         "noise_coef", "w_src", "w_hat", "w_tar", "coeff", "w_rec")]


_SIGS = {
    "hedit_last_error": (C.c_char_p, []),
    "hedit_version": (C.c_int, []),
    "hedit_unet_create": (C.c_int, [C.POINTER(UnetCfg), C.POINTER(C.c_void_p)]),
    "hedit_unet_destroy": (None, [C.c_void_p]),
    "hedit_unet_num_params": (C.c_int, [C.c_void_p]),
    "hedit_unet_param_name": (C.c_char_p, [C.c_void_p, C.c_int]),
    "hedit_unet_param_shape": (C.c_int, [C.c_void_p, C.c_int, C.POINTER(C.c_int), C.POINTER(C.c_int)]),
    "hedit_unet_load": (C.c_int, [C.c_void_p, C.c_char_p, C.c_void_p, C.c_size_t, C.c_void_p]),
    "hedit_unet_param_bf16_exact": (C.c_int, [C.c_void_p, C.c_int]),
    "hedit_unet_missing": (C.c_int, [C.c_void_p]),
    "hedit_unet_workspace_bytes": (C.c_size_t, [C.c_void_p, C.c_int, C.c_int, C.c_int]),
    "hedit_unet_forward": (C.c_int, [C.c_void_p, C.c_void_p, C.c_float, C.c_void_p, C.c_int, C.c_int,
                                     C.c_int, C.POINTER(P2PPlan), C.c_void_p, C.c_void_p, C.c_size_t,
                                     C.c_void_p]),
    "hedit_unet_forward_shared": (C.c_int, [C.c_void_p, C.c_void_p, C.c_int, C.POINTER(C.c_int), C.c_float, C.c_void_p, C.c_int,
                                            C.c_int, C.c_int, C.POINTER(P2PPlan), C.c_void_p, C.c_void_p, C.c_size_t, C.c_void_p]),
    "hedit_unet_set_attn_hook": (C.c_int, [C.c_void_p, C.c_void_p, C.c_void_p]),
    "hedit_unet_num_store_layers": (C.c_int, [C.c_void_p, C.c_int, C.c_int]),
    "hedit_unet_store_layer_info": (C.c_int, [C.c_void_p, C.c_int, C.c_int, C.c_int, C.POINTER(C.c_int),
                                              C.POINTER(C.c_int)]),
    "hedit_prof_enable": (C.c_int, [C.c_void_p, C.c_int, C.c_int]),
    "hedit_prof_reset": (C.c_int, [C.c_void_p]),
    "hedit_prof_collect": (C.c_int, [C.c_void_p, C.c_int, C.POINTER(C.c_double), C.POINTER(C.c_double),
                                     C.POINTER(C.c_int64)]),
    "hedit_prof_collect_bytes": (C.c_int, [C.c_void_p, C.c_int, C.POINTER(C.c_double)]),
    "hedit_prof_records": (C.c_int, [C.c_void_p, C.POINTER(C.c_double), C.c_int, C.POINTER(C.c_int)]),
    "hedit_step_base": (C.c_int, [C.c_void_p, C.c_void_p, C.c_void_p, C.c_void_p, C.c_int, C.c_int,
                                  C.c_int, C.POINTER(StepCoef), C.c_void_p]),
    "hedit_step_pair": (C.c_int, [C.c_void_p, C.c_void_p, C.c_void_p, C.c_void_p, C.c_void_p, C.c_int, C.c_int, C.c_int,
                                  C.POINTER(StepCoef), C.c_void_p]),
    "hedit_step_invert": (C.c_int, [C.c_void_p, C.c_void_p, C.c_void_p, C.c_void_p, C.c_void_p, C.c_int, C.c_int,
                                    C.POINTER(StepCoef), C.c_void_p]),
    "hedit_step_update": (C.c_int, [C.c_void_p, C.c_void_p, C.c_void_p, C.c_void_p, C.c_int64, C.c_void_p,
                                    C.c_void_p, C.c_void_p, C.c_int, C.c_int, C.c_int, C.POINTER(StepCoef),
                                    C.c_void_p]),
    "hedit_step_tweedie": (C.c_int, [C.c_void_p, C.c_void_p, C.c_int64, C.c_void_p, C.c_void_p, C.c_int, C.c_int,
                                     C.c_float, C.c_float, C.c_float, C.c_float, C.c_void_p]),
    "hedit_step_style": (C.c_int, [C.c_void_p, C.c_void_p, C.c_void_p, C.c_void_p, C.c_int64, C.c_void_p, C.c_void_p,
                                   C.c_void_p, C.c_int, C.c_int, C.c_float, C.c_float, C.c_float, C.c_float, C.c_void_p]),
    "hedit_local_blend": (C.c_int, [C.POINTER(C.c_void_p), C.c_int, C.c_int, C.c_void_p, C.c_void_p, C.c_void_p, C.c_int,
                                    C.c_int, C.c_int, C.c_int, C.c_float, C.c_void_p]),
    "hedit_local_blend_sub": (C.c_int, [C.POINTER(C.c_void_p), C.c_int, C.c_int, C.c_void_p, C.c_void_p, C.c_void_p, C.c_void_p,
                                        C.c_int, C.c_int, C.c_int, C.c_int, C.c_float, C.c_float, C.c_void_p]),
    "hedit_ddpm_create": (C.c_int, [C.POINTER(DdpmCfg), C.POINTER(C.c_void_p)]),
    "hedit_ddpm_destroy": (None, [C.c_void_p]),
    "hedit_ddpm_num_params": (C.c_int, [C.c_void_p]),
    "hedit_ddpm_param_name": (C.c_char_p, [C.c_void_p, C.c_int]),
    "hedit_ddpm_param_shape": (C.c_int, [C.c_void_p, C.c_int, C.POINTER(C.c_int), C.POINTER(C.c_int)]),
    "hedit_ddpm_load": (C.c_int, [C.c_void_p, C.c_char_p, C.c_void_p, C.c_size_t, C.c_void_p]),
# ... 106 lines not shown
    "hedit_axis_mix": (C.c_int, [C.c_void_p, C.c_void_p, C.c_void_p, C.c_void_p, C.c_int, C.c_int64, C.c_int, C.c_int, C.c_int,
                                 C.c_void_p]),
    "hedit_k_gemm_ws_bytes": (C.c_size_t, [C.c_int, C.c_int, C.c_int, C.c_int]),
    "hedit_k_gemm_canonical_chunk": (C.c_int, [C.c_int, C.c_int, C.c_int]),
    "hedit_k_gemm_plan_splits": (C.c_int, [C.c_int, C.c_int, C.c_int, C.c_int]),
    "hedit_k_gemm": (C.c_int, [C.c_void_p, C.c_void_p, C.c_void_p, C.c_void_p, C.c_void_p] + [C.c_int] * 13 +
                     [C.c_void_p, C.c_void_p]),
    "hedit_k_conv_gn": (C.c_int, [C.c_void_p, C.c_void_p, C.c_void_p, C.c_void_p, C.c_void_p] + [C.c_int] * 12 +
                        [C.c_void_p, C.c_void_p, C.c_void_p]),
    "hedit_k_groupnorm_from_parts": (C.c_int, [C.c_void_p, C.c_void_p, C.c_void_p, C.c_void_p, C.c_int, C.c_int, C.c_int, C.c_int,
                                               C.c_float, C.c_int, C.c_void_p, C.c_int, C.c_void_p, C.c_int, C.c_void_p, C.c_void_p]),
    "hedit_k_pack_geglu": (C.c_int, [C.c_void_p, C.c_void_p, C.c_void_p, C.c_void_p, C.c_int, C.c_int, C.c_void_p]),
    "hedit_k_gemm_geglu": (C.c_int, [C.c_void_p, C.c_void_p, C.c_void_p, C.c_void_p, C.c_int, C.c_int, C.c_int,
                                     C.c_int, C.c_int, C.c_void_p]),
    "hedit_test_set_flags": (C.c_int, [C.c_int]),
    "hedit_storage_is_f16": (C.c_int, []),
    "hedit_k_lin_chain_stream_bytes": (C.c_size_t, [C.c_int]),
    "hedit_k_lin_chain_pack": (C.c_int, [C.c_void_p, C.c_void_p, C.c_void_p, C.c_void_p, C.c_float, C.c_void_p, C.c_void_p]),
    "hedit_k_lin_chain": (C.c_int, [C.c_void_p, C.c_int64, C.c_void_p, C.c_int64, C.c_void_p, C.c_int, C.c_void_p, C.c_void_p, C.c_void_p,
                                    C.c_float, C.c_void_p, C.c_void_p, C.c_int64, C.c_void_p, C.c_int64, C.c_void_p, C.c_int64,
                                    C.c_void_p, C.c_int64, C.c_int, C.c_int, C.c_void_p]),
    "hedit_k_lin_chain_sched": (C.c_int, [C.c_void_p, C.c_int64, C.c_void_p, C.c_int64, C.c_void_p, C.c_int, C.c_void_p, C.c_void_p, C.c_void_p,
                                          C.c_float, C.c_void_p, C.c_void_p, C.c_int64, C.c_void_p, C.c_int64, C.c_void_p, C.c_int64,
                                          C.c_void_p, C.c_int64, C.c_int, C.c_int, C.c_int, C.c_void_p]),
    "hedit_k_groupnorm_affine": (C.c_int, [C.c_void_p, C.c_void_p, C.c_void_p, C.c_int, C.c_int, C.c_int, C.c_int, C.c_float, C.c_void_p,
                                           C.c_void_p, C.c_void_p]),
    "hedit_k_ffn_channels": (C.c_int, []),
    "hedit_k_ffn_stream_bytes": (C.c_size_t, [C.c_int]),
    "hedit_k_ffn_bias_bytes": (C.c_size_t, []),
    "hedit_k_ffn_pack": (C.c_int, [C.c_void_p, C.c_void_p, C.c_void_p, C.c_void_p, C.c_void_p, C.c_void_p, C.c_void_p, C.c_void_p]),
    "hedit_k_ffn_chain": (C.c_int, [C.c_void_p, C.c_int64, C.c_void_p, C.c_int64, C.c_void_p, C.c_int64, C.c_void_p, C.c_void_p, C.c_void_p,
                                    C.c_float, C.c_void_p, C.c_void_p, C.c_void_p, C.c_void_p, C.c_void_p, C.c_int64, C.c_int, C.c_int,
                                    C.c_void_p]),
    "hedit_k_ffn_fused": (C.c_int, [C.c_void_p, C.c_int64, C.c_void_p, C.c_void_p, C.c_float, C.c_void_p, C.c_void_p,
                                    C.c_void_p, C.c_void_p, C.c_int64, C.c_int, C.c_int, C.c_void_p]),
    "hedit_k_groupnorm_ws_bytes": (C.c_size_t, [C.c_int, C.c_int, C.c_int]),
    "hedit_k_groupnorm": (C.c_int, [C.c_void_p, C.c_void_p, C.c_void_p, C.c_void_p, C.c_int, C.c_int, C.c_int,
                                    C.c_int, C.c_float, C.c_int, C.c_void_p, C.c_void_p]),
    "hedit_k_layernorm": (C.c_int, [C.c_void_p, C.c_void_p, C.c_void_p, C.c_void_p, C.c_int64, C.c_int,
                                    C.c_float, C.c_void_p]),
    "hedit_k_geglu": (C.c_int, [C.c_void_p, C.c_void_p, C.c_int64, C.c_int, C.c_void_p]),
    "hedit_k_self_attn": (C.c_int, [C.c_void_p, C.c_int, C.c_void_p, C.c_int, C.c_void_p, C.c_int64, C.c_void_p,
                                    C.c_int, C.c_int, C.c_int, C.c_int, C.c_int, C.c_void_p, C.c_void_p, C.c_void_p]),
    "hedit_k_cross_attn": (C.c_int, [C.c_void_p, C.c_int, C.c_void_p, C.c_int, C.c_void_p, C.c_int64, C.c_void_p,
                                     C.c_int, C.c_int, C.c_int, C.c_int, C.c_int, C.POINTER(P2PPlan), C.c_void_p,
                                     C.c_void_p]),
    "hedit_k_attn_probs": (C.c_int, [C.c_void_p, C.c_int, C.c_void_p, C.c_int, C.c_void_p, C.c_int, C.c_int, C.c_int, C.c_int,
                                     C.c_int, C.c_int, C.c_void_p]),
    "hedit_k_attn_apply": (C.c_int, [C.c_void_p, C.c_void_p, C.c_int64, C.c_void_p, C.c_int, C.c_int, C.c_int, C.c_int, C.c_int,
                                     C.c_int, C.c_int, C.c_void_p]),
    "hedit_k_pack_conv3x3": (C.c_int, [C.c_void_p, C.c_void_p, C.c_int, C.c_int, C.c_void_p]),
    "hedit_k_f32_to_bf16": (C.c_int, [C.c_void_p, C.c_void_p, C.c_int64, C.c_void_p]),
    "hedit_k_groupnorm_stats": (C.c_int, [C.c_void_p, C.c_void_p, C.c_void_p, C.c_void_p, C.c_int, C.c_int, C.c_int,
                                          C.c_int, C.c_float, C.c_int, C.c_void_p, C.c_void_p, C.c_void_p]),
    "hedit_k_groupnorm_bwd_ws_bytes": (C.c_size_t, [C.c_int, C.c_int, C.c_int]),
    "hedit_k_groupnorm_bwd": (C.c_int, [C.c_void_p] * 7 + [C.c_int] * 5 + [C.c_void_p, C.c_void_p]),
    "hedit_k_softmax_rows": (C.c_int, [C.c_void_p, C.c_void_p, C.c_int64, C.c_int, C.c_float, C.c_void_p]),
    "hedit_k_softmax_blockdiag": (C.c_int, [C.c_void_p, C.c_void_p, C.c_int64, C.c_int, C.c_int, C.c_float, C.c_void_p]),
    "hedit_k_softmax_bwd": (C.c_int, [C.c_void_p, C.c_void_p, C.c_void_p, C.c_int64, C.c_int, C.c_float, C.c_void_p]),
    "hedit_k_transpose": (C.c_int, [C.c_void_p, C.c_void_p, C.c_int, C.c_int, C.c_void_p]),
    "hedit_k_sum2x2": (C.c_int, [C.c_void_p, C.c_void_p, C.c_int, C.c_int, C.c_int, C.c_int, C.c_void_p]),
    "hedit_k_pack_conv3x3_dgrad": (C.c_int, [C.c_void_p, C.c_void_p, C.c_int, C.c_int, C.c_void_p]),
    "hedit_k_pack_linear_t": (C.c_int, [C.c_void_p, C.c_void_p, C.c_int, C.c_int, C.c_void_p]),
    "hedit_k_flip_oihw": (C.c_int, [C.c_void_p, C.c_void_p, C.c_int, C.c_int, C.c_int, C.c_void_p]),
}

# ... 50 lines not shown
```

### h-edit_amd/hedit/engine.py

```python
import ctypes as C

import torch

from . import _lib


def _f(x):
    return float(x)


class Schedule:

    def __init__(self, scheduler):
        self.s = scheduler
        self.ab = scheduler.alphas_cumprod.float().cpu()
        self.final = scheduler.final_alpha_cumprod.float().cpu() if isinstance(
            scheduler.final_alpha_cumprod, torch.Tensor) else torch.tensor(float(scheduler.final_alpha_cumprod))
        self.T = scheduler.num_inference_steps
        self.n_train = scheduler.config.num_train_timesteps

    def ab_prev(self, t):
        p = t - self.n_train // self.T
        return self.ab[p] if p >= 0 else self.final

    def variance(self, t):
        a_t, a_p = self.ab[t], self.ab_prev(t)
        return ((1 - a_p) / (1 - a_t)) * (1 - a_t / a_p)

    def full_coeff(self, t, t_prev, eta, ddim_inv):
        ab = self.ab
        sig, a = (1 - ab) ** 0.5, ab ** 0.5
        omega = eta * (sig[t_prev] / (sig[t] * a[t_prev])) * ((ab[t_prev] - ab[t]) ** 0.5)
        if ddim_inv:
            omega = 0
        return (1 - ab[t_prev] - omega ** 2) ** 0.5

    def edit_coeff(self, t, t_prev, eta, ddim_inv):
        ab = self.ab
        ratio = (ab ** 0.5)[t_prev] / (ab ** 0.5)[t]
        return self.full_coeff(t, t_prev, eta, ddim_inv) - ((1 - ab) ** 0.5)[t] * ratio

    def step_coef(self, t, t_prev, eta, ddim_inv, cfg, w_rec=0.0, coeff=None):
        a_t, a_p = self.ab[t], self.ab_prev(t)
        var = self.variance(t)
        c = _lib.StepCoef()
        c.sqrt_ab_t = _f(a_t ** 0.5)
        c.sqrt_1m_ab_t = _f((1 - a_t) ** 0.5)
        c.sqrt_ab_prev = _f(a_p ** 0.5)
        c.dir_coef = _f((1 - a_p) ** 0.5) if ddim_inv else _f((1 - a_p - (eta ** 2) * var) ** 0.5)
        c.noise_coef = 0.0 if eta <= 0 else (_f(eta) if ddim_inv else _f(eta * var ** 0.5))
        c.w_src, c.w_hat, c.w_tar = (float(v) for v in cfg)
        c.coeff = _f(self.edit_coeff(t, t_prev, eta, ddim_inv)) if coeff is None else _f(coeff)
        c.w_rec = float(w_rec)
        return c


class HEditEngine:
    def __init__(self, model, share_latents=True):
        self.model = model
        self.share_latents = share_latents
        self.unet = model.unet
        self.lib = _lib.lib()
        self.dev = model.unet.device
        self.style_chunk = 8

    def step_base(self, eps, xt, z, out, n, rows, coef):
        elems = xt[0].numel()
        _lib.check(self.lib.hedit_step_base(_lib.ptr(eps), _lib.ptr(xt), _lib.ptr(z), _lib.ptr(out), n, elems,
                                            rows, C.byref(coef), _lib.cur_stream()))

    def step_update(self, e_u_src, e_c_src, e_u_tar, e_c_tar, x_k, x_base, out, n, k_gt0, coef):
        elems = x_k[0].numel()
        for t_ in (e_u_src, e_c_src, e_u_tar, e_c_tar, x_k, x_base, out):
            assert t_.is_contiguous() and t_.dtype == torch.float32
        _lib.check(self.lib.hedit_step_update(_lib.ptr(e_u_src), _lib.ptr(e_c_src), _lib.ptr(e_u_tar),
                                              _lib.ptr(e_c_tar), elems, _lib.ptr(x_k), _lib.ptr(x_base),
                                              _lib.ptr(out), n, elems, int(k_gt0), C.byref(coef),
                                              _lib.cur_stream()))

    def style_step(self, e_u_src, e_c_src, e_u_tar, e_c_tar, x, tt, cfg_scales, image_encoder, weight):
        vae = self.model.vae
        if vae is None:
            raise RuntimeError("style guidance needs model.vae (hedit.vae.AutoencoderKL)")
        n, elems = x.shape[0], x[0].numel()
        ab = float(self.model.scheduler.alphas_cumprod[tt])
        sab, s1m = ab ** 0.5, (1.0 - ab) ** 0.5
        inv_scale = 1.0 / 0.18215
# ... 34 lines not shown
            with torch.no_grad():
                return self.model.text_encoder(tok.input_ids)[0].float()
        out = []
        for p in prompts:
            tok = self.model.tokenizer([p], padding="max_length", max_length=self.model.tokenizer.model_max_length,
                                       truncation=True, return_tensors="pt")
            with torch.no_grad():
                out.append(self.model.text_encoder(tok.input_ids.to(self.dev))[0].float())
        return torch.cat(out)

    @torch.no_grad()
    def run(self, xT, zs, prompt_pairs, cfg_scales, controller=None, eta=1.0, p2p=True, implicit=True,
            K=1, w_rec=0.1, after_skip_steps=None, ddim_inv=False, ctx=None, fuse_src_pass=False,
            reuse_orig_eps=False, style=None, rec_pull=True):
        if style is not None and not (p2p and implicit):
            raise ValueError("style guidance is defined for the implicit P2P loop only (n-style h_edit.py)")
        sch = self.model.scheduler
        S = Schedule(sch)
        T = sch.num_inference_steps
        if after_skip_steps is None:
            after_skip_steps = T
        n = xT.shape[0]
        dev = self.dev
        xT = xT.to(device=dev, dtype=torch.float32)
        if zs is not None:
            zs = zs.to(device=dev, dtype=torch.float32).contiguous()
        if ctx is None:
            null = self.encode([""])
            src = self.encode([p[0] for p in prompt_pairs])
            tar = self.encode([p[1] for p in prompt_pairs])
        else:
            null, src, tar = (c.to(device=dev, dtype=torch.float32) for c in ctx)
        nulln = null.expand(n, -1, -1) if null.shape[0] == 1 else null
        ctx_base4 = torch.cat([nulln, nulln, src, src]).contiguous()
        ctx_base2 = torch.cat([nulln, src]).contiguous()
        ctx_edit = torch.cat([nulln, nulln, src, tar]).contiguous()
        ctx_src = src.contiguous()
        ctx_edit5 = torch.cat([nulln, nulln, src, tar, src]).contiguous() if fuse_src_pass else None

        ts = [int(v) for v in sch.timesteps]
        op = ts[-after_skip_steps:]
        ahead = ts[-(after_skip_steps + 1)] if after_skip_steps != T else -1
        xt = torch.cat([xT, xT]).contiguous()
        x_prev = torch.empty_like(xt)
        off = None

        from .p2p.ptp_classes import runs_in_python
        foreign = runs_in_python(controller)
        if foreign:
            if n != 1 or fuse_src_pass or reuse_orig_eps:
                raise ValueError("a foreign controller runs one image at a time, without fuse_src_pass / reuse_orig_eps "
                                 "(it sees the reference's 4-row batch)")
            if not callable(controller):
                raise TypeError("a foreign controller must be callable as controller(attn, is_cross, place_in_unet, save_attn)")
        step_cb = getattr(controller, "step_callback", None) if controller is not None else None
        if step_cb is not None and not callable(step_cb):
            raise TypeError("controller.step_callback must be callable as step_callback(x_t) -> x_t")

        share = self.share_latents

        def unet_rows(parts, blocks, t, ctx_rows, plan=None):
            if not share:
                return self.unet.forward_raw(torch.cat([parts[b] for b in blocks]), t, ctx_rows, plan)
            lat = parts[0] if len(parts) == 1 else torch.cat(parts)
            return self.unet.forward_raw(lat, t, ctx_rows, plan, row_latent=[b * n + j for b in blocks for j in range(n)])

        def p2p_pass(parts, blocks, t, save):
            rows = len(blocks) * n
            if foreign:
                return self.unet.forward_hooked(torch.cat([parts[b] for b in blocks]), t, ctx_edit, controller, save)
            plan = controller._plan(self.unet, rows, xT.shape[2], xT.shape[3], save) if controller is not None else None
            e = unet_rows(parts, blocks, t, ctx_edit5 if rows == 5 * n else ctx_edit, plan)
            if controller is not None:
                controller._after_pass(save)
            return e

        carry = None
        reuse = reuse_orig_eps and p2p and implicit
        for i, t in enumerate(op):
            idx = T - i - (T - after_skip_steps + 1)
            z = zs[idx] if zs is not None else None
            tt = op[i + 1] if i < len(op) - 1 else 0
            eta_i = float(eta[idx]) if isinstance(eta, (list, tuple)) else float(eta)
            coef = S.step_coef(t, tt, eta_i, ddim_inv, cfg_scales, w_rec)

            if (not p2p) and implicit and i == 0 and ahead != -1:
                xe = xt[n:]
                e = unet_rows([xe], (0, 0, 0, 0), t, ctx_edit, off)
                c0 = S.step_coef(t, tt, eta_i, ddim_inv, cfg_scales, w_rec, coeff=S.edit_coeff(ahead, t, eta_i, ddim_inv))
                new = torch.empty_like(xe)
                self.step_update(e[0:n], e[2 * n:3 * n], e[n:2 * n], e[3 * n:], xe, xe, new, n, False, c0)
                xt = torch.cat([xt[:n], new]).contiguous()

            if p2p and reuse and carry is not None:
                e2 = unet_rows([xt[n:]], (0, 0), t, ctx_base2, off)
                e = torch.cat([carry[0], e2[:n], carry[1], e2[n:]])
                self.step_base(e, xt, z, x_prev, n, 4, coef)
            elif p2p:
                e = unet_rows([xt[:n], xt[n:]], (0, 1, 0, 1), t, ctx_base4, off)
                self.step_base(e, xt, z, x_prev, n, 4, coef)
            else:
                e = unet_rows([xt[n:]], (0, 0), t, ctx_base2, off)
                self.step_base(e, xt, z, x_prev, n, 2, coef)
            x_orig, x_base = x_prev[:n], x_prev[n:]

            if not implicit:
                new = torch.empty_like(x_base)
                if p2p:
                    e_src = self.unet.forward_raw(xt[n:].contiguous(), t, ctx_src, off)
                    e = p2p_pass([xt[:n], xt[n:]], (0, 1, 0, 1), t, True)
                    self.step_update(e[n:2 * n], e_src, e[n:2 * n], e[3 * n:], x_base, x_base, new, n, False, coef)
                else:
                    e = unet_rows([xt[n:]], (0, 0, 0, 0), t, ctx_edit, off)
                    self.step_update(e[0:n], e[2 * n:3 * n], e[n:2 * n], e[3 * n:], x_base, x_base, new, n, False, coef)
                x_k = new
            else:
                x_k = x_base.clone()
                for k in range(K):
                    new = torch.empty_like(x_k)
                    if p2p:
                        save = not (k < K - 1 and K > 1)
                        if fuse_src_pass:
                            e = p2p_pass([x_orig, x_k], (0, 1, 0, 1, 1), tt, save)
                            e_src = e[4 * n:]
                        else:
                            e_src = self.unet.forward_raw(x_k, tt, ctx_src, off)
                            e = p2p_pass([x_orig, x_k], (0, 1, 0, 1), tt, save)
                        self.step_update(e[n:2 * n], e_src, e[n:2 * n], e[3 * n:4 * n], x_k, x_base, new, n,
                                         k > 0 and style is None and rec_pull, coef)
                        if style is not None and style[0] is not None:
                            with torch.enable_grad():
                                new = self.style_step(e[n:2 * n], e_src, e[n:2 * n], e[3 * n:4 * n], new, tt, cfg_scales,
                                                      style[0], style[1])
                        if reuse:
                            carry = (e[0:n], e[2 * n:3 * n])
                    else:
                        e = unet_rows([x_k], (0, 0, 0, 0), tt, ctx_edit, off)
                        self.step_update(e[0:n], e[2 * n:3 * n], e[n:2 * n], e[3 * n:], x_k, x_base, new, n, k > 0, coef)
                    x_k = new

            xt = torch.cat([x_orig, x_k]).contiguous()
            if step_cb is not None:
                xt = step_cb(xt)
        return xt[n:].clone(), xt[:n].clone()

    @torch.no_grad()
    def run_pnp(self, xT, zs, prompts, cfg_scales, eta=1.0, K=1, after_skip_steps=None, ddim_inv=True):
        from .plug_n_play.pnp_utils import register_time
        sch = self.model.scheduler
        S = Schedule(sch)
        T = sch.num_inference_steps
        if after_skip_steps is None:
            after_skip_steps = T
        dev = self.dev
        xT = xT.to(device=dev, dtype=torch.float32)
        n = xT.shape[0]
        pairs = [list(prompts[:2])] if isinstance(prompts[0], str) else [list(p[:2]) for p in prompts]
        if len(pairs) != n:
            raise ValueError("one [source, target] prompt pair per image expected")
        if zs is not None:
            zs = zs.to(device=dev, dtype=torch.float32).contiguous()
            if zs.dim() == 4:
                zs = zs[:, None]
        null = self.encode([""]).expand(n, -1, -1)
        src, tar = self.encode([p[0] for p in pairs]), self.encode([p[1] for p in pairs])
        ctx_base4 = torch.cat([null, null, src, src]).contiguous()
        ctx_k2 = torch.cat([null, src]).contiguous()
        ctx_pair = torch.cat([src, tar]).contiguous()
        editor = getattr(self.unet, "_attention_editor", None)
        ts = [int(v) for v in sch.timesteps]
        op = ts[-after_skip_steps:]
        xt = torch.cat([xT, xT]).contiguous()
        x_prev = torch.empty_like(xt)
        H, W = xT.shape[2], xT.shape[3]
        for i, t in enumerate(op):
            idx = T - i - (T - after_skip_steps + 1)
            z = zs[idx] if zs is not None else None
            tt = op[i + 1] if i < len(op) - 1 else 0
            eta_i = float(eta[idx]) if isinstance(eta, (list, tuple)) else float(eta)
            coef = S.step_coef(t, tt, eta_i, ddim_inv, cfg_scales, 0.0)
            register_time(self.model, t)
            e = self.unet.forward_raw(torch.cat([xt, xt]), t, ctx_base4, None)
            self.step_base(e, xt, z, x_prev, n, 4, coef)
            x_orig, x_base = x_prev[:n], x_prev[n:]
            x_k = x_base.clone()
            for _ in range(K):
                register_time(self.model, tt)
                e2 = self.unet.forward_raw(torch.cat([x_k, x_k]), tt, ctx_k2, None)
                plan = editor._plan(self.unet, 2 * n, H, W, True, n_images=n) if editor is not None else None
                ep = self.unet.forward_raw(torch.cat([x_orig, x_k]), tt, ctx_pair, plan)
                if editor is not None:
                    editor._after_pass(True)
                new = torch.empty_like(x_k)
                self.step_update(e2[0:n], e2[n:2 * n], e2[0:n], ep[n:2 * n].contiguous(), x_k, x_base, new, n, False, coef)
                x_k = new
            xt = torch.cat([x_orig, x_k]).contiguous()
        return xt[n:].clone(), xt[:n].clone()

    def step_pair(self, e_u, e_c, xt, z, out, n, kinds, coefs):
        elems = xt[0].numel()
        for t_ in (e_u, e_c, xt, out) + (() if z is None else (z,)):
            assert t_.is_contiguous() and t_.dtype == torch.float32
        arr = (_lib.StepCoef * kinds)(*coefs)
        _lib.check(self.lib.hedit_step_pair(_lib.ptr(e_u), _lib.ptr(e_c), _lib.ptr(xt), _lib.ptr(z), _lib.ptr(out), n, elems,
                                            kinds, arr, _lib.cur_stream()))

    def _pair_coefs(self, S, t, eta_i, ddim_inv, cfg_pair):
        return [S.step_coef(t, 0, eta_i, ddim_inv, (cfg_pair[0], 0.0, 0.0), coeff=0.0),
                S.step_coef(t, 0, 0.0 if ddim_inv else eta_i, ddim_inv, (cfg_pair[-1], 0.0, 0.0), coeff=0.0)]

    @torch.no_grad()
    def run_direct(self, xT, zs, prompt_pairs, cfg_pair, controller=None, eta=1.0, after_skip_steps=None, ddim_inv=False,
                   control=True):
        sch = self.model.scheduler
        S = Schedule(sch)
        T = sch.num_inference_steps
        if after_skip_steps is None:
            after_skip_steps = T
        n = xT.shape[0]
        dev = self.dev
        pairs = [list(p) for p in prompt_pairs]
        if len(pairs) != n or any(len(p) != len(pairs[0]) or len(p) not in (1, 2) for p in pairs):
            raise ValueError("one [source, target] pair (or one [target]) per image expected")
        kinds = len(pairs[0])
        if len(cfg_pair) != kinds:
            raise ValueError("one guidance weight per prompt expected")
        xT = xT.to(device=dev, dtype=torch.float32)
        if zs is not None:
            zs = zs.to(device=dev, dtype=torch.float32).contiguous()
        null = self.encode([""]).expand(n, -1, -1)
        tar = self.encode([p[-1] for p in pairs])
        if kinds == 2:
            ctx = torch.cat([null, null, self.encode([p[0] for p in pairs]), tar]).contiguous()
        else:
            ctx = torch.cat([null, tar]).contiguous()
        controlled = control and kinds == 2 and controller is not None

        from .p2p.ptp_classes import runs_in_python
        foreign = controlled and runs_in_python(controller)
        if foreign:
            if n != 1:
                raise ValueError("a foreign controller runs one image at a time (it sees the reference's 4-row batch)")
            if not callable(controller):
                raise TypeError("a foreign controller must be callable as controller(attn, is_cross, place_in_unet, save_attn)")
        step_cb = getattr(controller, "step_callback", None) if controller is not None else None
        if step_cb is not None and not callable(step_cb):
            raise TypeError("controller.step_callback must be callable as step_callback(x_t) -> x_t")

        ts = [int(v) for v in sch.timesteps]
        op = ts[-after_skip_steps:]
        xt = torch.cat([xT] * kinds).contiguous()
        H, W = xT.shape[2], xT.shape[3]
        for i, t in enumerate(op):
            idx = T - i - (T - after_skip_steps + 1)
            z = zs[idx] if zs is not None else None
            eta_i = float(eta[idx]) if isinstance(eta, (list, tuple)) else float(eta)
            x_in = torch.cat([xt, xt])
            if foreign:
                e = self.unet.forward_hooked(x_in, t, ctx, controller, True)
            elif controlled:
                e = self.unet.forward_raw(x_in, t, ctx, controller._plan(self.unet, 4 * n, H, W, True))
                controller._after_pass(True)
            else:
                e = self.unet.forward_raw(x_in, t, ctx, None)
            coefs = self._pair_coefs(S, t, eta_i, ddim_inv, cfg_pair)
            x_next = torch.empty_like(xt)
            self.step_pair(e[:kinds * n], e[kinds * n:], xt, z, x_next, n, kinds, coefs[:kinds])
            xt = x_next
            if kinds == 2 and step_cb is not None:
                xt = step_cb(xt)
        if kinds == 1:
            if step_cb is not None:
                xt = step_cb(xt)
            return xt.clone(), None
        return xt[n:].clone(), xt[:n].clone()

    @torch.no_grad()
    def run_direct_pnp(self, xT, zs, prompts, cfg_pair, eta=0.0, after_skip_steps=None, ddim_inv=False, uncond="null"):
        from .plug_n_play.pnp_utils import register_time
        if uncond not in ("null", "src"):
            raise ValueError("uncond must be 'null' or 'src'")
        sch = self.model.scheduler
        S = Schedule(sch)
        T = sch.num_inference_steps
        if after_skip_steps is None:
            after_skip_steps = T
        dev = self.dev
        xT = xT.to(device=dev, dtype=torch.float32)
        n = xT.shape[0]
        pairs = [list(prompts[:2])] if isinstance(prompts[0], str) else [list(p[:2]) for p in prompts]
        if len(pairs) != n:
            raise ValueError("one [source, target] prompt pair per image expected")
        if zs is not None:
            zs = zs.to(device=dev, dtype=torch.float32).contiguous()
            if zs.dim() == 4:
                zs = zs[:, None]
        src, tar = self.encode([p[0] for p in pairs]), self.encode([p[1] for p in pairs])
        u = src if uncond == "src" else self.encode([""]).expand(n, -1, -1)
        ctx_u = torch.cat([u, u]).contiguous()
        ctx_pair = torch.cat([src, tar]).contiguous()
        editor = getattr(self.unet, "_attention_editor", None)
        ts = [int(v) for v in sch.timesteps]
        op = ts[-after_skip_steps:]
        xt = torch.cat([xT, xT]).contiguous()
        H, W = xT.shape[2], xT.shape[3]
        for i, t in enumerate(op):
            idx = T - i - (T - after_skip_steps + 1)
            z = zs[idx] if zs is not None else None
            eta_i = float(eta[idx]) if isinstance(eta, (list, tuple)) else float(eta)
            register_time(self.model, t)
            e_u = self.unet.forward_raw(xt, t, ctx_u, None)
            plan = editor._plan(self.unet, 2 * n, H, W, True, n_images=n) if editor is not None else None
            e_c = self.unet.forward_raw(xt, t, ctx_pair, plan)
            if editor is not None:
                editor._after_pass(True)
            x_next = torch.empty_like(xt)
            self.step_pair(e_u, e_c, xt, z, x_next, n, 2, self._pair_coefs(S, t, eta_i, ddim_inv, cfg_pair))
            xt = x_next
        return xt[n:].clone(), xt[:n].clone()

    @torch.no_grad()
    def ddpm_inversion(self, x0, prompts, eta=1.0, cfg_src=1.0, noise=None, generator=None, return_noise=False):
        sch = self.model.scheduler
        S = Schedule(sch)
        T = sch.num_inference_steps
        dev = self.dev
        x0 = x0.to(device=dev, dtype=torch.float32)
        n = x0.shape[0]
        elems = x0[0].numel()
        ts = [int(v) for v in sch.timesteps]
        ab = S.ab
        xts = torch.zeros(T + 1, *x0.shape, device=dev)
        nzs = torch.zeros(T + 1, *x0.shape, device=dev) if return_noise else None
        xts[0] = x0
        for j, t in enumerate(reversed(ts)):
            idx = j + 1
            if noise is not None:
                nz = noise[idx].to(dev)
            else:
                nz = torch.randn(x0.shape, device=dev, generator=generator)
            if nzs is not None:
                nzs[idx] = nz
            xts[idx] = x0 * _f(ab[t] ** 0.5) + nz * _f((1 - ab[t]) ** 0.5)
        null = self.encode([""]).expand(n, -1, -1)
        cond = any(p != "" for p in prompts)
        ctx = torch.cat([null, self.encode(list(prompts))]).contiguous() if cond else null.contiguous()
        zs = torch.zeros(T, *x0.shape, device=dev)
        for i, t in enumerate(ts):
            idx = T - i - 1
            xt = xts[idx + 1]
            if cond:
                if self.share_latents:
                    e = self.unet.forward_raw(xt, t, ctx, row_latent=list(range(n)) * 2)
                else:
                    e = self.unet.forward_raw(torch.cat([xt, xt]), t, ctx)
                e_u, e_c = e[:n], e[n:]
            else:
                e_u = e_c = self.unet.forward_raw(xt.contiguous(), t, ctx)
            eta_i = float(eta[idx]) if isinstance(eta, (list, tuple)) else float(eta)
            coef = S.step_coef(t, 0, eta_i, False, (cfg_src, 0.0, 0.0), coeff=0.0)
            _lib.check(self.lib.hedit_step_invert(_lib.ptr(e_u), _lib.ptr(e_c), _lib.ptr(xt), _lib.ptr(xts[idx]),
                                                  _lib.ptr(zs[idx]), n, elems, C.byref(coef), _lib.cur_stream()))
        if return_noise:
            return zs, xts, nzs
        return zs, xts

    @torch.no_grad()
    def ddim_inversion(self, w0, prompts, cfg_scale):
        sch = self.model.scheduler
        S = Schedule(sch)
        T = sch.num_inference_steps
        step = S.n_train // T
        dev = self.dev
        lat = w0.to(device=dev, dtype=torch.float32).clone()
        n = lat.shape[0]
        ts = [int(v) for v in sch.timesteps]
        null = self.encode([""]).expand(n, -1, -1)
        ctx = torch.cat([null, self.encode(list(prompts))]).contiguous()
        ab = S.ab
# ... 29 lines not shown
```

### h-edit_amd/hedit/unet.py

```python
import ctypes as C
import hashlib
import math

import torch

from . import _lib

SD15_CONFIG = dict(in_channels=4, out_channels=4, sample_size=64,
                   block_out_channels=(320, 640, 1280, 1280),
                   down_block_types=("CrossAttnDownBlock2D", "CrossAttnDownBlock2D",
                                     "CrossAttnDownBlock2D", "DownBlock2D"),
                   up_block_types=("UpBlock2D", "CrossAttnUpBlock2D", "CrossAttnUpBlock2D",
                                   "CrossAttnUpBlock2D"),
                   layers_per_block=2, cross_attention_dim=768, attention_head_dim=8,
                   norm_num_groups=32)

TINY_CONFIG = dict(in_channels=4, out_channels=4, sample_size=32,
                   block_out_channels=(64, 128, 128),
                   down_block_types=("CrossAttnDownBlock2D", "CrossAttnDownBlock2D", "DownBlock2D"),
                   up_block_types=("UpBlock2D", "CrossAttnUpBlock2D", "CrossAttnUpBlock2D"),
                   layers_per_block=2, cross_attention_dim=64, attention_head_dim=2,
                   norm_num_groups=32)


class UNetOutput(dict):
    @property
    def sample(self):
        return self["sample"]


class AttnProcessor:
    controller = None


def random_state_dict(param_shapes, seed=0):
    sd = {}
    for name, shape in param_shapes.items():
        hsh = hashlib.sha256(f"{seed}:{name}".encode()).digest()
        g = torch.Generator().manual_seed(int.from_bytes(hsh[:7], "little"))
        if len(shape) >= 2:
            fan_in = 1
            for s in shape[1:]:
                fan_in *= s
            sd[name] = torch.randn(shape, generator=g) / math.sqrt(fan_in)
        elif "norm" in name and name.endswith("weight"):
            sd[name] = 1.0 + 0.1 * torch.randn(shape, generator=g)
        elif "norm" in name:
            sd[name] = 0.1 * torch.randn(shape, generator=g)
        else:
            sd[name] = 0.02 * torch.randn(shape, generator=g)
    return sd


class UNet2DConditionModel:
    def __init__(self, config=None, device="cuda:0"):
        cfg = dict(SD15_CONFIG)
        cfg.update(config or {})
        self.config = cfg
        self.device = torch.device(device)
        if self.device.type != "cuda":
            raise RuntimeError("hedit.UNet2DConditionModel runs on the GPU only (HIP kernels)")
        self.in_channels = cfg["in_channels"]
        self.sample_size = cfg["sample_size"]
        self._lib = _lib.lib()
        c = _lib.UnetCfg()
# ... 130 lines not shown
    PROF_KINDS = ("conv3x3_gemm", "linear_gemm", "self_attn", "cross_attn", "norm", "other")

    def prof_enable(self, on, max_records=8192):
        _lib.check(self._lib.hedit_prof_enable(self._h, int(on), max_records))

    def prof_reset(self):
        _lib.check(self._lib.hedit_prof_reset(self._h))

    def prof_collect(self):
        torch.cuda.synchronize(self.device)
        out = {}
        ms, fl, n = C.c_double(), C.c_double(), C.c_int64()
        for i, k in enumerate(self.PROF_KINDS):
            _lib.check(self._lib.hedit_prof_collect(self._h, i, C.byref(ms), C.byref(fl), C.byref(n)))
            out[k] = (ms.value, fl.value, n.value)
        return out

    def prof_collect_bytes(self):
        out = {}
        b = C.c_double()
        for i, k in enumerate(self.PROF_KINDS):
            _lib.check(self._lib.hedit_prof_collect_bytes(self._h, i, C.byref(b)))
            out[k] = b.value
        return out

    def prof_records(self, max_rows=16384):
        import numpy as np
        torch.cuda.synchronize(self.device)
        rows = np.zeros((max_rows, 8), dtype=np.float64)
        n = C.c_int()
        _lib.check(self._lib.hedit_prof_records(self._h, rows.ctypes.data_as(C.POINTER(C.c_double)), max_rows, C.byref(n)))
        return rows[:n.value]

    def forward_raw(self, sample, t, ctx, plan=None, out=None, row_latent=None):
        B, Cc, H, W = sample.shape
        if row_latent is not None:
            B = len(row_latent)
        if sample.dtype != torch.float32 or ctx.dtype != torch.float32:
            raise TypeError("sample and encoder_hidden_states must be float32")
        if ctx.shape != (B, 77, self.config["cross_attention_dim"]):
            raise ValueError(f"encoder_hidden_states must be ({B}, 77, {self.config['cross_attention_dim']}), "
                             f"got {tuple(ctx.shape)}")
        sample = sample.contiguous()
        ctx = ctx.contiguous()
        if out is None:
            out = torch.empty(B, self.config["out_channels"], H, W, dtype=torch.float32, device=sample.device)
        ws = self._workspace(B, H, W)
        if row_latent is None:
            _lib.check(self._lib.hedit_unet_forward(
                self._h, _lib.ptr(sample), C.c_float(float(t)), _lib.ptr(ctx), B, H, W,
                C.byref(plan) if plan is not None else None, _lib.ptr(out), _lib.ptr(ws), ws.numel(),
                _lib.cur_stream()))
            return out
        if sample.data_ptr() % 16:
            sample = sample.clone()
        _lib.check(self._lib.hedit_unet_forward_shared(
            self._h, _lib.ptr(sample), sample.shape[0], (C.c_int * B)(*row_latent), C.c_float(float(t)), _lib.ptr(ctx), B, H, W,
            C.byref(plan) if plan is not None else None, _lib.ptr(out), _lib.ptr(ws), ws.numel(),
            _lib.cur_stream()))
        return out

    _HOOK_T = C.CFUNCTYPE(C.c_int, C.c_void_p, C.c_void_p, C.c_int, C.c_int, C.c_int, C.c_int, C.c_int, C.c_int, C.c_void_p)

    def forward_hooked(self, sample, t, ctx, controller, save_attn=True, out=None):
        B, _, H, W = sample.shape
        state = {"exc": None}
        places = ("down", "mid", "up")

        def cb(_user, probs, bh, nq, nk, is_cross, place, _layer, _stream):
            try:
                off = int(probs) - self._ws.data_ptr()
                view = self._ws[off:off + bh * nq * nk * 4].view(torch.float32).view(bh, nq, nk)
                attn = view.clone()
                controller(attn, bool(is_cross), places[place], save_attn)
                view.copy_(attn)
                return 0
            except BaseException as e:
                state["exc"] = e
                return 1

        fn = self._HOOK_T(cb)
        _lib.check(self._lib.hedit_unet_set_attn_hook(self._h, C.cast(fn, C.c_void_p), None))
        try:
            try:
                return self.forward_raw(sample, t, ctx, None, out)
            except _lib.HipError:
                if state["exc"] is not None:
                    raise state["exc"]
                raise
        finally:
            _lib.check(self._lib.hedit_unet_set_attn_hook(self._h, None, None))

    def forward(self, sample, timestep=None, encoder_hidden_states=None, cross_attention_kwargs=None,
                return_dict=True):
        kw = dict(cross_attention_kwargs or {})
        use_controller = kw.pop("use_controller", True)
        save_attn = kw.pop("save_attn", True)
        use_editor = kw.pop("use_editor", True)
        if kw:
            raise TypeError(f"unsupported cross_attention_kwargs {sorted(kw)}")
        if isinstance(timestep, torch.Tensor):
            tt = timestep.reshape(-1)
            if tt.numel() > 1 and not bool((tt == tt[0]).all()):
                raise NotImplementedError("per-sample timesteps: the batch must share one timestep")
            t = float(tt[0])
        else:
            t = float(timestep)
        sample = sample.to(device=self.device, dtype=torch.float32)
        ctx = encoder_hidden_states.to(device=self.device, dtype=torch.float32)
        controller = self._controller() if use_controller else None
        if controller is None and use_editor:
            controller = getattr(self, "_attention_editor", None)
        from .p2p.ptp_classes import runs_in_python
        if runs_in_python(controller):
            return UNetOutput(sample=self.forward_hooked(sample, t, ctx, controller, save_attn))
        plan = None
        if controller is not None:
# ... 8 lines not shown
```

### include/hedit.h

```cpp
#ifndef HEDIT_H
#define HEDIT_H
#include <stddef.h>
#include <stdint.h>

#ifdef __cplusplus
extern "C" {
#endif

#define HEDIT_MAX_LEVELS 8

typedef struct hedit_unet hedit_unet;

typedef struct {
  int in_channels, out_channels, sample_size;
  int n_levels;
  int block_out_channels[HEDIT_MAX_LEVELS];
  int down_has_attn[HEDIT_MAX_LEVELS];
  int up_has_attn[HEDIT_MAX_LEVELS];
  int layers_per_block;
  int cross_attention_dim;
  int heads;
  int norm_num_groups;
} hedit_unet_cfg;

// ... 11 lines not shown
  int n_store;
  const int32_t* kv_src;
  int kv_first_block;
  int qk_first_block, qk_max_tokens;
  const int32_t* feat_src;
  int feat_resblock;
  float* const* h_store_self;
  int n_store_self;
} hedit_p2p_plan;

typedef struct {
  float sqrt_ab_t, sqrt_1m_ab_t, sqrt_ab_prev, dir_coef, noise_coef;
  float w_src, w_hat, w_tar, coeff, w_rec;
} hedit_step_coef;

const char* hedit_last_error(void);
int hedit_version(void);

int hedit_unet_create(const hedit_unet_cfg* cfg, hedit_unet** out);
void hedit_unet_destroy(hedit_unet* h);
int hedit_unet_num_params(const hedit_unet* h);
const char* hedit_unet_param_name(const hedit_unet* h, int i);
int hedit_unet_param_shape(const hedit_unet* h, int i, int* ndim, int* dims4);
int hedit_unet_load(hedit_unet* h, const char* name, const float* w, size_t numel, void* stream);
int hedit_unet_param_bf16_exact(const hedit_unet* h, int i);
int hedit_unet_missing(const hedit_unet* h);
size_t hedit_unet_workspace_bytes(hedit_unet* h, int B, int height, int width);
int hedit_unet_forward(hedit_unet* h, const float* x, float t, const float* ctx, int B, int height,
                       int width, const hedit_p2p_plan* plan, float* eps_out, void* workspace,
                       size_t workspace_bytes, void* stream);
int hedit_unet_forward_shared(hedit_unet* h, const float* x, int D, const int* row_latent, float t, const float* ctx, int B,
                              int height, int width, const hedit_p2p_plan* plan, float* eps_out, void* workspace,
                              size_t workspace_bytes, void* stream);
typedef int (*hedit_attn_hook_fn)(void* user, float* probs, int batch_heads, int n_query, int n_key, int is_cross, int place,
                                  int layer, void* stream);
int hedit_unet_set_attn_hook(hedit_unet* h, hedit_attn_hook_fn fn, void* user);
int hedit_unet_num_store_layers(const hedit_unet* h, int height, int width);
int hedit_unet_store_layer_info(const hedit_unet* h, int height, int width, int i, int* tokens,
                                int* place );

int hedit_prof_enable(hedit_unet* h, int on, int max_records);
int hedit_prof_reset(hedit_unet* h);
int hedit_prof_collect(hedit_unet* h, int kind, double* total_ms, double* total_flops, int64_t* count);
int hedit_prof_collect_bytes(hedit_unet* h, int kind, double* total_bytes);
int hedit_prof_records(hedit_unet* h, double* rows, int max_rows, int* n_rows);

int hedit_step_base(const float* eps, const float* xt, const float* z, float* x_prev, int n_img,
                    int elems, int eps_rows_per_img, const hedit_step_coef* c, void* stream);
int hedit_step_pair(const float* e_u, const float* e_c, const float* xt, const float* z, float* x_next, int n_img,
                    int elems, int n_kinds, const hedit_step_coef* c, void* stream);
int hedit_step_invert(const float* e_u, const float* e_c, const float* xt, float* x_prev, float* z_out,
                      int n_img, int elems, const hedit_step_coef* c, void* stream);
int hedit_step_update(const float* e_u_src, const float* e_c_src, const float* e_u_tar,
                      const float* e_c_tar, int64_t stride_img, const float* x_k,
                      const float* x_base, float* x_out, int n_img, int elems, int k_gt0,
                      const hedit_step_coef* c, void* stream);
int hedit_step_tweedie(const float* e_u_tar, const float* e_c_tar, int64_t stride_img, const float* x, float* z0,
                       int n_img, int elems, float w_tar, float sqrt_ab, float sqrt_1m_ab, float inv_scale, void* stream);
int hedit_step_style(const float* e_u_src, const float* e_c_src, const float* e_u_tar, const float* e_c_tar,
                     int64_t stride_img, const float* x, const float* g_z, float* x_out, int n_img, int elems,
                     float w_hat, float w_tar, float chain, float weight, void* stream);
int hedit_axis_mix(const float* in, float* out, const int32_t* idx, const float* val, int nnz, int64_t outer, int n_in, int n_out,
                   int inner, void* stream);
int hedit_local_blend(float* const* h_maps, int n_maps, int heads, const float* alpha_layers,
                      const int32_t* enabled, float* xt, int n_img, int C, int H, int W, float th,
                      void* stream);
// ... 24 lines not shown
                         float* d_z, float* image, void* workspace, size_t workspace_bytes, void* stream);
int hedit_vae_decode_keep(hedit_vae* h, const float* z, int B, int latent_h, int latent_w, float* image,
                          void* workspace, size_t workspace_bytes, void* stream);
int hedit_vae_decode_backward(hedit_vae* h, const float* d_image, float* d_z, void* workspace, void* stream);
int hedit_vae_encode(hedit_vae* h, const float* image, int B, int height, int width, float* mean,
                     void* workspace, size_t workspace_bytes, void* stream);

size_t hedit_k_gemm_ws_bytes(int M, int N, int K, int splits);
int hedit_k_gemm_canonical_chunk(int M_nominal, int N_nominal, int K);
int hedit_k_gemm_plan_splits(int M, int N, int K, int chunk_kt);
int hedit_k_gemm(const void* A, const void* W, const float* bias, const void* residual, void* C,
                 int M, int N, int K, int lda, int ldc, int ldr, int mode, int Hin, int Win,
                 int Cin, int Hout, int Wout, int splits, void* partial_ws, void* stream);
int hedit_k_conv_gn(const void* A, const void* W, const float* bias, const void* residual, void* C, int M, int N, int K, int ldc,
                    int ldr, int mode, int Hin, int Win, int Cin, int Hout, int Wout, int splits, void* partial_ws, float* gn_part,
                    void* stream);
int hedit_k_groupnorm_from_parts(const void* x, void* y, const float* gamma, const float* beta, int B, int HW, int C, int G,
                                 float eps, int silu, const float* part_a, int ca, const float* part_b, int cb, void* ws,
                                 void* stream);
int hedit_k_pack_geglu(const float* w, const float* bias, void* w_packed_bf16, float* bias_packed,
                       int inner, int K, void* stream);
int hedit_k_gemm_geglu(const void* A, const void* w_packed, const float* bias_packed, void* C, int M,
                       int inner, int K, int lda, int ldc, void* stream);
int hedit_k_ffn_channels(void);
size_t hedit_k_ffn_stream_bytes(int with_outer_layers);
size_t hedit_k_ffn_bias_bytes(void);
int hedit_k_ffn_pack(const float* w1, const float* b1, const float* w2, const float* w_pre, const float* w_post, void* stream_out,
                     float* bias1_out, void* stream);
int hedit_k_ffn_fused(const void* x, int64_t ldx, const float* gamma, const float* beta, float eps, const void* w_stream,
                      const float* bias1_packed, const float* bias2, void* out, int64_t ldo, int M, int C, void* stream);
int hedit_k_ffn_chain(const void* a, int64_t lda, const void* t1, int64_t ldt1, const void* x, int64_t ldx, const float* bias_pre,
                      const float* gamma, const float* beta, float eps, const void* w_stream, const float* bias1_packed,
                      const float* bias2, const float* bias_post, void* out, int64_t ldo, int M, int C, void* stream);
size_t hedit_k_lin_chain_stream_bytes(int n_out);
int hedit_k_lin_chain_pack(const float* w_pre, const float* w0, const float* w1, const float* w2, float scale0, void* stream_out,
                           void* stream);
int hedit_k_lin_chain(const void* a, int64_t lda, const void* r1, int64_t ldr1, const float* gn_ss, int rows_per_image,
                      const float* bias_pre, const float* gamma, const float* beta, float eps, const void* w_stream, void* out_mid,
                      int64_t ldmid, void* out_q, int64_t ldq, void* out_k, int64_t ldk, void* out, int64_t ldo, int M, int C,
                      void* stream);
int hedit_k_lin_chain_sched(const void* a, int64_t lda, const void* r1, int64_t ldr1, const float* gn_ss, int rows_per_image,
                            const float* bias_pre, const float* gamma, const float* beta, float eps, const void* w_stream, void* out_mid,
                            int64_t ldmid, void* out_q, int64_t ldq, void* out_k, int64_t ldk, void* out, int64_t ldo, int M, int C,
                            int sched, void* stream);
int hedit_storage_is_f16(void);
int hedit_test_set_flags(int flags);
size_t hedit_k_groupnorm_ws_bytes(int B, int HW, int C);
int hedit_k_groupnorm_affine(const void* x, const float* gamma, const float* beta, int B, int HW, int C, int G, float eps, void* ws,
                             float* ss_out, void* stream);
int hedit_k_groupnorm(const void* x, void* y, const float* gamma, const float* beta, int B, int HW,
                      int C, int G, float eps, int silu, void* ws, void* stream);
int hedit_k_layernorm(const void* x, void* y, const float* gamma, const float* beta, int64_t rows,
                      int C, float eps, void* stream);
int hedit_k_geglu(const void* x, void* y, int64_t rows, int inner, void* stream);
int hedit_k_self_attn(const void* q, int ldq, const void* k, int ldk, const void* vt, int64_t ldvt,
                      void* out, int ldo, int B, int N, int heads, int d, const int32_t* qk_src, const int32_t* kv_src,
                      void* stream);
int hedit_k_cross_attn(const void* q, int ldq, const void* k, int ldk, const void* vt, int64_t ldvt,
                       void* out, int ldo, int B, int N, int heads, int d,
                       const hedit_p2p_plan* plan, float* store, void* stream);
int hedit_k_attn_probs(const void* q, int ldq, const void* k, int ldk, float* probs, int B, int N, int M, int kstride,
                       int heads, int d, void* stream);
int hedit_k_attn_apply(const float* probs, const void* vt, int64_t ldvt, void* out, int ldo, int B, int N, int M,
                       int kstride, int heads, int d, void* stream);
int hedit_k_pack_conv3x3(const float* w_oihw, void* out, int O, int I, void* stream);
int hedit_k_f32_to_bf16(const float* x, void* y, int64_t n, void* stream);
// ... 147 lines not shown
```

Before: 2.589.

## Precompute cross-attention context projections once and map shared-stem rows in-kernel

```diff
diff --git a/h-edit_amd/csrc/attn.hip b/h-edit_amd/csrc/attn.hip
--- a/h-edit_amd/csrc/attn.hip
+++ b/h-edit_amd/csrc/attn.hip
@@ -603,7 +603,7 @@
 };
 
 template <int D>
-__global__ __launch_bounds__(256, (D <= 80 ? 2 : 1)) void cross_attn_kernel(CrossAttnParams p) {
+__global__ __launch_bounds__(256, (D <= 80 ? 2 : 1)) void cross_attn_kernel(CrossAttnParams p, RowMapArg qmap) {
   using H = HeadCfg<D>;
   using S = CrossSmem<D>;
   extern __shared__ __attribute__((aligned(16))) char smem[];
@@ -654,6 +654,7 @@
   };
 
   auto load_q = [&](int b, bf16x8* qf) {
+    if (p.q_map) b = rowmap_at(qmap, __builtin_amdgcn_readfirstlane(b));
     const bf16_t* qp = p.q + ((long)b * p.N + (q_ok ? q_row : 0)) * p.ldq + h * D;
 #pragma unroll
     for (int ks = 0; ks < H::DK; ++ks) {
@@ -793,7 +794,10 @@
   using S = CrossSmem<D>;
   if (int rc = hedit_dyn_lds(reinterpret_cast<const void*>(&cross_attn_kernel<D>), S::TOTAL)) return rc;
   dim3 grid(cdiv(p.N, 128), p.heads, p.n_pairs + p.n_single);
-  hipLaunchKernelGGL((cross_attn_kernel<D>), grid, dim3(256), S::TOTAL, st, p);
+  RowMapArg qmap;
+  if (p.q_map) qmap.m = *p.q_map;
+  else qmap.m = RowMap{};
+  hipLaunchKernelGGL((cross_attn_kernel<D>), grid, dim3(256), S::TOTAL, st, p, qmap);
   LAUNCH_CHECK();
   return HEDIT_OK;
 }
@@ -955,6 +959,7 @@
 int cross_attn_launch(const CrossAttnParams& p, hipStream_t st) {
   ARG_CHECK(p.n_pairs + p.n_single > 0, "cross_attn: nothing to do");
   ARG_CHECK(p.ldq % 8 == 0 && p.ldk % 8 == 0 && p.ldvt % 8 == 0 && p.ldo % 4 == 0, "cross_attn: strides");
+  ARG_CHECK(!p.q_map || p.B <= HEDIT_ROWMAP_MAX, "cross_attn: image map");
   switch (p.d) {
     case 32: return launch_cross<32>(p, st);
     case 40: return launch_cross<40>(p, st);
diff --git a/h-edit_amd/csrc/c_api.hip b/h-edit_amd/csrc/c_api.hip
--- a/h-edit_amd/csrc/c_api.hip
+++ b/h-edit_amd/csrc/c_api.hip
@@ -252,6 +252,30 @@
   return ffn_fused_launch(f, S(stream));
 } catch (...) { return hedit_abi_catch(); }
 
+int hedit_k_ffn_chain_mapped(const void* a, int64_t lda, const void* t1, int64_t ldt1, const void* x, int64_t ldx,
+                             const float* bias_pre, const float* gamma, const float* beta, float eps, const void* w_stream,
+                             const float* bias1_packed, const float* bias2, const float* bias_post, void* out, int64_t ldo, int M,
+                             int C, const int* image_map, int n_images, int src_images, int rows_per_image, void* stream) try {
+  ARG_CHECK(a && t1 && x && image_map, "ffn_chain args");
+  ARG_CHECK(n_images >= 1 && n_images <= HEDIT_ROWMAP_MAX && rows_per_image > 0 && (long)n_images * rows_per_image == M,
+            "ffn_chain: image map");
+  RowMap map{};
+  for (int i = 0; i < n_images; ++i) {
+    ARG_CHECK(image_map[i] >= 0 && image_map[i] < src_images, "ffn_chain: image_map entries must lie in [0, src_images)");
+    map.src[i] = (uint16_t)image_map[i];
+  }
+  FfnParams f{};
+  f.a = reinterpret_cast<const bf16_t*>(a); f.lda = (long)lda;
+  f.x = reinterpret_cast<const bf16_t*>(t1); f.ldx = (long)ldt1;
+  f.r2 = reinterpret_cast<const bf16_t*>(x); f.ldr2 = (long)ldx;
+  f.bias_pre = bias_pre; f.bias_post = bias_post;
+  f.gamma = gamma; f.beta = beta; f.eps = eps;
+  f.stream = reinterpret_cast<const bf16_t*>(w_stream); f.bias1p = bias1_packed; f.bias2 = bias2;
+  f.out = reinterpret_cast<bf16_t*>(out); f.ldo = (long)ldo; f.M = M; f.C = C;
+  f.map = &map; f.rows_per_image = rows_per_image;
+  return ffn_fused_launch(f, S(stream));
+} catch (...) { return hedit_abi_catch(); }
+
 int hedit_k_ffn_chain(const void* a, int64_t lda, const void* t1, int64_t ldt1, const void* x, int64_t ldx, const float* bias_pre,
                       const float* gamma, const float* beta, float eps, const void* w_stream, const float* bias1_packed, const float* bias2,
                       const float* bias_post, void* out, int64_t ldo, int M, int C, void* stream) try {
@@ -297,7 +321,7 @@
 int hedit_storage_is_f16(void) { return HEDIT_F16; }
 
 int hedit_test_set_flags(int flags) try {
-  ARG_CHECK(flags >= 0 && flags <= 15, "hedit_test_set_flags: bit 0 drained ring waits, bit 1 exact self-attention pass, bit 2 pixel-UNet GroupNorm statistics path flipped, bit 3 no persistent linear kernel");
+  ARG_CHECK(flags >= 0 && flags <= 63, "hedit_test_set_flags: bit 0 drained ring waits, bit 1 exact self-attention pass, bit 2 pixel-UNet GroupNorm statistics path flipped, bit 3 no persistent linear kernel, bit 4 prepared contexts recomputed per call, bit 5 shared-stem results copied per row");
   g_test_flags.store(flags, std::memory_order_relaxed);
   return HEDIT_OK;
 } catch (...) { return hedit_abi_catch(); }
diff --git a/h-edit_amd/csrc/ffn.hip b/h-edit_amd/csrc/ffn.hip
--- a/h-edit_amd/csrc/ffn.hip
+++ b/h-edit_amd/csrc/ffn.hip
@@ -107,6 +107,8 @@
   const float* bias_post;
   bf16_t* out; long ldo;
   int M;
+  int rows_per_image;
+  RowMapArg map;
 };
 
 template <class F, int... I>
@@ -183,7 +185,6 @@
   const int m_wave = blockIdx.x * BLOCK_ROWS + wave * ROWS_PER_WAVE;
   int row_c = m_wave + lm;
   if (row_c > p.M - 1) row_c = p.M - 1;
-
 #if defined(__HIP_DEVICE_COMPILE__)
   const __amdgpu_buffer_rsrc_t rs_w = __builtin_amdgcn_make_buffer_rsrc(const_cast<bf16_t*>(p.stream), (short)0, (int)(stream_iters(PRE, POST) * ITER_BYTES), 0x00020000);
   const __amdgpu_buffer_rsrc_t rs_b = __builtin_amdgcn_make_buffer_rsrc(const_cast<float*>(p.bias1p), (short)0, (int)BIAS_BYTES, 0x00020000);
@@ -249,8 +250,14 @@
     asm volatile("s_nop 3" ::: "memory");
   };
 
+  int row_shift = 0;
+  if (p.rows_per_image > 0) {
+    const int img = __builtin_amdgcn_readfirstlane((m_wave < p.M ? m_wave : p.M - 1) / p.rows_per_image);
+    row_shift = __builtin_amdgcn_readfirstlane((rowmap_at(p.map, img) - img) * p.rows_per_image);
+  }
+
   bf16x8 Xn[FKS];
-  load_rows(p.r1, p.ldr1, PRE ? p.bias_pre : nullptr);
+  load_rows(p.r1 + (long)row_shift * p.ldr1, p.ldr1, PRE ? p.bias_pre : nullptr);
   if constexpr (PRE) {
     const bf16_t* src = p.a + (long)row_c * p.lda + hi * 8;
 #pragma unroll
@@ -461,7 +468,7 @@
   if constexpr (POST) {
     settle();
     frags_from_acc(std::false_type{}, 0.f, 1.f);
-    load_rows(p.r2, p.ldr2, p.bias_post);
+    load_rows(p.r2 + (long)row_shift * p.ldr2, p.ldr2, p.bias_post);
     publish();
     asm volatile("s_waitcnt vmcnt(0)" ::: "memory");
 #pragma unroll
@@ -546,12 +553,19 @@
   ARG_CHECK(f.x && f.out && f.stream && f.bias1p && f.bias2 && f.gamma && f.beta, "ffn: null");
   const bool pre = f.a != nullptr, post = f.r2 != nullptr;
   ARG_CHECK(pre == post, "ffn: the chain exists with both outer linear layers or with neither");
+  ARG_CHECK(pre || !f.map, "ffn: an image map goes with the outer linear layers");
   ChainKernelParams k{};
   k.r1 = f.x; k.ldr1 = f.ldx; k.gamma = f.gamma; k.beta = f.beta; k.eps = f.eps;
   k.stream = f.stream; k.bias1p = f.bias1p; k.bias2 = f.bias2; k.out = f.out; k.ldo = f.ldo; k.M = f.M;
   if (pre) {
     ARG_CHECK(f.lda % 8 == 0 && f.ldr2 % 4 == 0 && f.ldx % 4 == 0 && f.bias_pre && f.bias_post, "ffn chain: alignment / biases");
     k.a = f.a; k.lda = f.lda; k.r2 = f.r2; k.ldr2 = f.ldr2; k.bias_pre = f.bias_pre; k.bias_post = f.bias_post;
+    if (f.map) {
+      ARG_CHECK(f.rows_per_image > 0 && f.rows_per_image % ROWS_PER_WAVE == 0 && f.M % f.rows_per_image == 0 &&
+                f.M / f.rows_per_image <= HEDIT_ROWMAP_MAX, "ffn chain: image map");
+      k.rows_per_image = f.rows_per_image;
+      k.map.m = *f.map;
+    }
     return launch_chain<true, true>(k, st);
   }
   return launch_chain<false, false>(k, st);
diff --git a/h-edit_amd/csrc/kernels.h b/h-edit_amd/csrc/kernels.h
--- a/h-edit_amd/csrc/kernels.h
+++ b/h-edit_amd/csrc/kernels.h
@@ -44,6 +44,13 @@
 bool pconv_supported(const GemmParams& p, int splits, int bn);
 int pconv_launch(const GemmParams& p, int bn, hipStream_t st);
 
+#define HEDIT_ROWMAP_MAX 512
+struct RowMap { uint16_t src[HEDIT_ROWMAP_MAX]; };
+union RowMapArg { RowMap m; uint32_t w[HEDIT_ROWMAP_MAX / 2]; };
+#if defined(__HIPCC__)
+__device__ __forceinline__ int rowmap_at(const RowMapArg& a, int i) { return (int)((a.w[i >> 1] >> ((i & 1) * 16)) & 0xffffu); }
+#endif
+
 struct FfnParams {
   const bf16_t* x; long ldx;
   const float* gamma; const float* beta; float eps;
@@ -55,6 +62,7 @@
   const bf16_t* a; long lda;
   const bf16_t* r2; long ldr2;
   const float* bias_pre; const float* bias_post;
+  const RowMap* map; int rows_per_image;
 };
 struct LinChainParams {
   const bf16_t* a; long lda;
@@ -100,8 +108,6 @@
 int splitk_reduce_ln_launch(const float* partial, int splits, const float* bias, const bf16_t* residual, int ldr, bf16_t* out,
                             bf16_t* y, const float* gamma, const float* beta, long rows, int C, float eps, hipStream_t st);
 int geglu_launch(const bf16_t* x, bf16_t* y, long rows, int inner, hipStream_t st);
-#define HEDIT_ROWMAP_MAX 512
-struct RowMap { uint16_t src[HEDIT_ROWMAP_MAX]; };
 int concat_launch(const bf16_t* a, int ca, const bf16_t* b, int cb, bf16_t* y, long rows, hipStream_t st,
                   const RowMap* b_map = nullptr, int rows_per_image = 0);
 int gather_rows_launch(const void* const* src, void* const* dst, int n, int B, long row_bytes, const RowMap& map, hipStream_t st);
@@ -163,6 +169,7 @@
   float* store;
   const int* singles;
   int n_single;
+  const RowMap* q_map;
 };
 int cross_attn_launch(const CrossAttnParams& p, hipStream_t st);
 
diff --git a/h-edit_amd/csrc/unet.hip b/h-edit_amd/csrc/unet.hip
--- a/h-edit_amd/csrc/unet.hip
+++ b/h-edit_amd/csrc/unet.hip
@@ -1,4 +1,5 @@
 #include <array>
+#include <atomic>
 #include <map>
 #include <string>
 #include <vector>
@@ -78,7 +79,8 @@
   void* hook_user = nullptr;
   bf16_t *wk2_all = nullptr, *wv2_all = nullptr;
   int ctx_n = 0, ctx_next = 0;
-  std::map<std::array<int, 4>, size_t> ws_cache;
+  std::map<std::array<int, 5>, size_t> ws_cache;
+  uint64_t epoch = 0;
 };
 
 namespace {
@@ -224,7 +226,6 @@
   Arena ar;
   const hedit_p2p_plan* plan;
   const float* temb_all;
-  const bf16_t* ctxb;
   const bf16_t* k2_all = nullptr;
   const bf16_t* vt2_all = nullptr;
   int store_idx = 0;
@@ -506,7 +507,7 @@
 }
 
 int transformer_rest(Fwd& f, const Attn& a, const bf16_t* x, bf16_t* t1, bf16_t* q2, int H, int W, bf16_t** out,
-                     bf16_t* dst = nullptr, int ldd = 0) {
+                     bf16_t* dst = nullptr, int ldd = 0, bool per_latent = false) {
   const int C = a.C, N = H * W, B = f.B, heads = f.h->cfg.heads, d = C / heads;
   const size_t M = (size_t)B * N;
   const hedit_p2p_plan* pl = (f.plan && f.plan->mode > 0) ? f.plan : nullptr;
@@ -521,6 +522,7 @@
     CrossAttnParams cp{};
     cp.q = q2; cp.ldq = C; cp.k = k2; cp.ldk = ldk2; cp.vt = vt2; cp.ldvt = MC; cp.out = ao; cp.ldo = C;
     cp.B = B; cp.N = N; cp.heads = heads; cp.d = d;
+    cp.q_map = per_latent ? f.map : nullptr;
     const bool stored_layer = N <= 1024;
     if (pl) {
       cp.n_pairs = pl->n_pairs; cp.pair_src = pl->pair_src; cp.pair_tar = pl->pair_tar;
@@ -550,6 +552,7 @@
     fp.bias_pre = a.o2_b; fp.bias_post = a.pout_b;
     fp.gamma = a.ln3g; fp.beta = a.ln3b; fp.eps = 1e-5f;
     fp.stream = a.ffs; fp.bias1p = a.ff1_bp; fp.bias2 = a.ff2_b; fp.out = y; fp.ldo = dst ? ldd : C; fp.M = (int)M; fp.C = C;
+    if (per_latent) { fp.map = f.map; fp.rows_per_image = N; }
     {
       ProfScope ps(f, PK_LINEAR, 2.0 * M * 14.0 * C * C, 8.0 * M * C + 28.0 * C * C);
       chain_prof(f, ps, M, C, 14, 128);
@@ -609,6 +612,8 @@
   return true;
 }
 
+inline bool test_stem_copies() { return (hedit_test_flags() & 32) != 0; }
+
 int broadcast_stem(Fwd& f, size_t row_elems, bf16_t** x, bf16_t** t1, bf16_t** q2, int D) {
   bf16_t** narrow[3] = {x, t1, q2};
   bf16_t* wide[3];
@@ -630,9 +635,34 @@
   return HEDIT_OK;
 }
 
+int project_context(Fwd& f, const float* ctx, bf16_t* ctxb, bf16_t* k2a, bf16_t* vt2a) {
+  hedit_unet* h = f.h;
+  const int dim = h->cfg.cross_attention_dim, MC = f.B * HEDIT_CTXP;
+  RUN(f, ctx_pad_launch(ctx, ctxb, f.B, dim, f.st));
+  TRY(linear(f, ctxb, MC, dim, h->wk2_all, h->ctx_n, nullptr, nullptr, k2a, h->ctx_n));
+  TRY(linear(f, h->wv2_all, h->ctx_n, dim, ctxb, MC, nullptr, nullptr, vt2a, MC, 2));
+  return HEDIT_OK;
+}
+
+int context_impl(hedit_unet* h, const float* ctx, int B, bf16_t* k2a, bf16_t* vt2a, void* ws, size_t ws_bytes, hipStream_t st,
+                 bool dry, size_t* peak) {
+  Fwd f;
+  f.h = h; f.B = B; f.st = st; f.plan = nullptr;
+  f.ar.base = reinterpret_cast<char*>(ws); f.ar.cap = ws_bytes; f.ar.dry = dry;
+  bf16_t* ctxb;
+  TRY(aalloc(f, &ctxb, (size_t)B * HEDIT_CTXP * h->cfg.cross_attention_dim));
+  TRY(project_context(f, ctx, ctxb, k2a, vt2a));
+  f.ar.free(ctxb);
+  if (peak) *peak = f.ar.peak;
+  return HEDIT_OK;
+}
+
+inline bool test_plain_context() { return (hedit_test_flags() & 16) != 0; }
+
 int forward_impl(hedit_unet* h, const float* x, float t, const float* ctx, int B, int H0, int W0,
                  const hedit_p2p_plan* plan, float* eps_out, void* ws, size_t ws_bytes, hipStream_t st,
-                 bool dry, size_t* peak, int D = 0, const RowMap* map = nullptr) {
+                 bool dry, size_t* peak, int D = 0, const RowMap* map = nullptr, bool prepared = false,
+                 const bf16_t* k2_prep = nullptr, const bf16_t* vt2_prep = nullptr) {
   const hedit_unet_cfg& c = h->cfg;
   Fwd f;
   f.h = h; f.B = B; f.st = st; f.plan = plan; f.map = map;
@@ -644,17 +674,17 @@
     return HEDIT_ERR_ARG;
   }
 
-  bf16_t* ctxb;
-  TRY(aalloc(f, &ctxb, (size_t)B * HEDIT_CTXP * c.cross_attention_dim));
-  RUN(f, ctx_pad_launch(ctx, ctxb, B, c.cross_attention_dim, st));
-  f.ctxb = ctxb;
-  {
+  if (prepared) {
+    f.k2_all = k2_prep;
+    f.vt2_all = vt2_prep;
+  } else {
+    bf16_t* ctxb;
+    TRY(aalloc(f, &ctxb, (size_t)B * HEDIT_CTXP * c.cross_attention_dim));
     const int MC = B * HEDIT_CTXP;
     bf16_t *k2a, *vt2a;
     TRY(aalloc(f, &k2a, (size_t)MC * h->ctx_n));
     TRY(aalloc(f, &vt2a, (size_t)MC * h->ctx_n));
-    TRY(linear(f, ctxb, MC, c.cross_attention_dim, h->wk2_all, h->ctx_n, nullptr, nullptr, k2a, h->ctx_n));
-    TRY(linear(f, h->wv2_all, h->ctx_n, c.cross_attention_dim, ctxb, MC, nullptr, nullptr, vt2a, MC, 2));
+    TRY(project_context(f, ctx, ctxb, k2a, vt2a));
     f.k2_all = k2a;
     f.vt2_all = vt2a;
   }
@@ -706,10 +736,11 @@
         }
       }
       cur = y;
-      if (stem) TRY(broadcast_stem(f, (size_t)H * W * blk.ch, &cur, &t1, &q2, D));
+      const bool mapped = stem && blk.attn[j].ffs != nullptr && (H * W) % 32 == 0 && !test_stem_copies();
+      if (stem && !mapped) TRY(broadcast_stem(f, (size_t)H * W * blk.ch, &cur, &t1, &q2, D));
       if (blk.has_attn) {
         bf16_t* z;
-        TRY(transformer_rest(f, blk.attn[j], cur, t1, q2, H, W, &z));
+        TRY(transformer_rest(f, blk.attn[j], cur, t1, q2, H, W, &z, nullptr, 0, mapped));
         f.ar.free(cur);
         cur = z;
       }
@@ -821,6 +852,8 @@
 
 }
 
+static std::atomic<uint64_t> g_weights_epoch{0};
+
 extern "C" {
 
 int hedit_unet_create(const hedit_unet_cfg* cfg, hedit_unet** out) try {
@@ -1005,6 +1038,7 @@
     TRY(pack_conv3x3_launch(w, reinterpret_cast<bf16_t*>(s.dst), s.O, s.I, st));
   }
   s.loaded = true;
+  h->epoch = ++g_weights_epoch;
   return HEDIT_OK;
 } catch (...) { return hedit_abi_catch(); }
 
@@ -1015,23 +1049,69 @@
   return m;
 } catch (...) { return hedit_abi_catch(); }
 
-size_t hedit_unet_workspace_bytes(hedit_unet* h, int B, int height, int width) try {
+static size_t workspace_need(hedit_unet* h, int B, int height, int width, bool prepared) {
   if (!h) return 0;
-  const std::array<int, 4> key{B, height, width, h->hook ? 1 : 0};
+  const std::array<int, 5> key{B, height, width, (h->hook ? 1 : 0) | (test_stem_copies() ? 2 : 0), prepared ? 1 : 0};
   auto it = h->ws_cache.find(key);
   if (it != h->ws_cache.end()) return it->second;
   size_t need = 0;
   for (int D = 0; D <= (B <= HEDIT_ROWMAP_MAX ? B : 0); ++D) {
     size_t peak = 0;
-    if (forward_impl(h, nullptr, 0.f, nullptr, B, height, width, nullptr, nullptr, nullptr, 0, nullptr, true, &peak, D) != HEDIT_OK) return 0;
+    if (forward_impl(h, nullptr, 0.f, nullptr, B, height, width, nullptr, nullptr, nullptr, 0, nullptr, true, &peak, D, nullptr,
+                     prepared) != HEDIT_OK) return 0;
     if (peak > need) need = peak;
   }
   need += 4096;
   h->ws_cache[key] = need;
   return need;
+}
+
+size_t hedit_unet_workspace_bytes(hedit_unet* h, int B, int height, int width) try {
+  return workspace_need(h, B, height, width, false);
 } catch (...) { (void)hedit_abi_catch(); return 0; }
 
-static int forward_checks(hedit_unet* h, const float* x, const float* ctx, int B, int height, int width, const hedit_p2p_plan* plan,
+size_t hedit_unet_workspace_bytes_prepared(hedit_unet* h, int B, int height, int width) try {
+  return workspace_need(h, B, height, width, true);
+} catch (...) { (void)hedit_abi_catch(); return 0; }
+
+static size_t context_half_bytes(const hedit_unet* h, int B) {
+  return (((size_t)B * HEDIT_CTXP * h->ctx_n * sizeof(bf16_t)) + 255) & ~(size_t)255;
+}
+
+size_t hedit_unet_context_bytes(const hedit_unet* h, int B) try {
+  if (!h || B < 1) return 0;
+  return 2 * context_half_bytes(h, B);
+} catch (...) { (void)hedit_abi_catch(); return 0; }
+
+size_t hedit_unet_context_workspace_bytes(hedit_unet* h, int B) try {
+  if (!h || B < 1) return 0;
+  size_t peak = 0;
+  if (context_impl(h, nullptr, B, nullptr, nullptr, nullptr, 0, nullptr, true, &peak) != HEDIT_OK) return 0;
+  return peak + 4096;
+} catch (...) { (void)hedit_abi_catch(); return 0; }
+
+int hedit_unet_context_prepare(hedit_unet* h, const float* ctx, int B, void* buf, size_t buf_bytes, void* workspace,
+                               size_t workspace_bytes, void* stream, hedit_unet_context* out) try {
+  ARG_CHECK(h && ctx && buf && workspace && out, "null");
+  ARG_CHECK(B >= 1, "B");
+  ARG_CHECK(reinterpret_cast<uintptr_t>(buf) % 256 == 0, "the context buffer must be 256-byte aligned");
+  if (hedit_unet_missing(h) != 0) {
+    hedit_set_error("UNet has " + std::to_string(hedit_unet_missing(h)) + " unloaded parameters");
+    return HEDIT_ERR_STATE;
+  }
+  const size_t half = context_half_bytes(h, B);
+  if (buf_bytes < 2 * half) {
+    hedit_set_error("context buffer too small (need " + std::to_string(2 * half) + " bytes)");
+    return HEDIT_ERR_ARG;
+  }
+  bf16_t* k2a = reinterpret_cast<bf16_t*>(buf);
+  bf16_t* vt2a = reinterpret_cast<bf16_t*>(reinterpret_cast<char*>(buf) + half);
+  TRY(context_impl(h, ctx, B, k2a, vt2a, workspace, workspace_bytes, reinterpret_cast<hipStream_t>(stream), false, nullptr));
+  out->buf = buf; out->bytes = 2 * half; out->B = B; out->ctx_n = h->ctx_n; out->storage_f16 = HEDIT_F16; out->epoch = h->epoch;
+  return HEDIT_OK;
+} catch (...) { return hedit_abi_catch(); }
+
+static int forward_checks(hedit_unet* h, const float* x, const void* ctx, int B, int height, int width, const hedit_p2p_plan* plan,
                           float* eps_out, void* workspace) {
   ARG_CHECK(h && x && ctx && eps_out && workspace, "null");
   ARG_CHECK(B >= 1, "B");
@@ -1051,19 +1131,31 @@
   return HEDIT_OK;
 }
 
-int hedit_unet_forward(hedit_unet* h, const float* x, float t, const float* ctx, int B, int height, int width,
-                       const hedit_p2p_plan* plan, float* eps_out, void* workspace, size_t workspace_bytes,
-                       void* stream) try {
-  TRY(forward_checks(h, x, ctx, B, height, width, plan, eps_out, workspace));
-  return forward_impl(h, x, t, ctx, B, height, width, plan, eps_out, workspace, workspace_bytes,
-                      reinterpret_cast<hipStream_t>(stream), false, nullptr);
-} catch (...) { return hedit_abi_catch(); }
-
-int hedit_unet_forward_shared(hedit_unet* h, const float* x, int D, const int* row_latent, float t, const float* ctx, int B,
-                              int height, int width, const hedit_p2p_plan* plan, float* eps_out, void* workspace,
-                              size_t workspace_bytes, void* stream) try {
-  TRY(forward_checks(h, x, ctx, B, height, width, plan, eps_out, workspace));
-  ARG_CHECK(row_latent && D >= 1 && D <= 65535, "row map");
+int hedit_unet_forward_prepared(hedit_unet* h, const float* x, int D, const int* row_latent, float t, const float* ctx,
+                                const hedit_unet_context* prepared, int B, int height, int width, const hedit_p2p_plan* plan,
+                                float* eps_out, void* workspace, size_t workspace_bytes, void* stream) try {
+  TRY(forward_checks(h, x, ctx ? static_cast<const void*>(ctx) : static_cast<const void*>(prepared), B, height, width, plan, eps_out,
+                     workspace));
+  const bf16_t *k2 = nullptr, *vt2 = nullptr;
+  if (prepared && test_plain_context()) {
+    ARG_CHECK(ctx, "the plain-context test switch needs the context tensor beside the prepared one");
+    prepared = nullptr;
+  }
+  if (prepared) {
+    ARG_CHECK(prepared->buf && prepared->B == B, "prepared context: made for another batch size B");
+    ARG_CHECK(prepared->storage_f16 == HEDIT_F16, "prepared context: made in the other storage format");
+    ARG_CHECK(prepared->epoch == h->epoch && prepared->ctx_n == h->ctx_n,
+              "prepared context: made before the last weight load (or by another UNet); prepare it again");
+    const size_t half = context_half_bytes(h, B);
+    ARG_CHECK(prepared->bytes == 2 * half, "prepared context: buffer size");
+    k2 = reinterpret_cast<const bf16_t*>(prepared->buf);
+    vt2 = reinterpret_cast<const bf16_t*>(reinterpret_cast<const char*>(prepared->buf) + half);
+  }
+  hipStream_t st = reinterpret_cast<hipStream_t>(stream);
+  if (!row_latent)
+    return forward_impl(h, x, t, ctx, B, height, width, plan, eps_out, workspace, workspace_bytes, st, false, nullptr, 0, nullptr,
+                        prepared != nullptr, k2, vt2);
+  ARG_CHECK(D >= 1 && D <= 65535, "row map");
   if (B > HEDIT_ROWMAP_MAX) {
     hedit_set_error("batch larger than " + std::to_string(HEDIT_ROWMAP_MAX) + " rows (the row map of shared latents)");
     return HEDIT_ERR_ARG;
@@ -1074,8 +1166,25 @@
     ARG_CHECK(row_latent[r] >= 0 && row_latent[r] < D, "row_latent entries must lie in [0, D)");
     map.src[r] = (uint16_t)row_latent[r];
   }
-  return forward_impl(h, x, t, ctx, B, height, width, plan, eps_out, workspace, workspace_bytes,
-                      reinterpret_cast<hipStream_t>(stream), false, nullptr, D, &map);
+  return forward_impl(h, x, t, ctx, B, height, width, plan, eps_out, workspace, workspace_bytes, st, false, nullptr, D, &map,
+                      prepared != nullptr, k2, vt2);
+} catch (...) { return hedit_abi_catch(); }
+
+int hedit_unet_forward(hedit_unet* h, const float* x, float t, const float* ctx, int B, int height, int width,
+                       const hedit_p2p_plan* plan, float* eps_out, void* workspace, size_t workspace_bytes,
+                       void* stream) try {
+  ARG_CHECK(ctx, "null");
+  return hedit_unet_forward_prepared(h, x, 0, nullptr, t, ctx, nullptr, B, height, width, plan, eps_out, workspace, workspace_bytes,
+                                     stream);
+} catch (...) { return hedit_abi_catch(); }
+
+int hedit_unet_forward_shared(hedit_unet* h, const float* x, int D, const int* row_latent, float t, const float* ctx, int B,
+                              int height, int width, const hedit_p2p_plan* plan, float* eps_out, void* workspace,
+                              size_t workspace_bytes, void* stream) try {
+  ARG_CHECK(ctx, "null");
+  ARG_CHECK(row_latent, "row map");
+  return hedit_unet_forward_prepared(h, x, D, row_latent, t, ctx, nullptr, B, height, width, plan, eps_out, workspace,
+                                     workspace_bytes, stream);
 } catch (...) { return hedit_abi_catch(); }
 
 int hedit_prof_enable(hedit_unet* h, int on, int max_records) try {
diff --git a/h-edit_amd/hedit/_lib.py b/h-edit_amd/hedit/_lib.py
--- a/h-edit_amd/hedit/_lib.py
+++ b/h-edit_amd/hedit/_lib.py
@@ -52,6 +52,11 @@
                 ("kv_src", C.c_void_p), ("kv_first_block", C.c_int),
                 ("qk_first_block", C.c_int), ("qk_max_tokens", C.c_int), ("feat_src", C.c_void_p), ("feat_resblock", C.c_int),
                 ("h_store_self", C.POINTER(C.c_void_p)), ("n_store_self", C.c_int)]
+
+
+class UnetContext(C.Structure):
+    _fields_ = [("buf", C.c_void_p), ("bytes", C.c_size_t), ("B", C.c_int), ("ctx_n", C.c_int), ("storage_f16", C.c_int),
+                ("reserved", C.c_int), ("epoch", C.c_uint64)]
 
 
 class StepCoef(C.Structure):
@@ -76,6 +81,14 @@
                                      C.c_void_p]),
     "hedit_unet_forward_shared": (C.c_int, [C.c_void_p, C.c_void_p, C.c_int, C.POINTER(C.c_int), C.c_float, C.c_void_p, C.c_int,
                                             C.c_int, C.c_int, C.POINTER(P2PPlan), C.c_void_p, C.c_void_p, C.c_size_t, C.c_void_p]),
+    "hedit_unet_context_bytes": (C.c_size_t, [C.c_void_p, C.c_int]),
+    "hedit_unet_context_workspace_bytes": (C.c_size_t, [C.c_void_p, C.c_int]),
+    "hedit_unet_context_prepare": (C.c_int, [C.c_void_p, C.c_void_p, C.c_int, C.c_void_p, C.c_size_t, C.c_void_p, C.c_size_t,
+                                             C.c_void_p, C.POINTER(UnetContext)]),
+    "hedit_unet_forward_prepared": (C.c_int, [C.c_void_p, C.c_void_p, C.c_int, C.POINTER(C.c_int), C.c_float, C.c_void_p,
+                                              C.POINTER(UnetContext), C.c_int, C.c_int, C.c_int, C.POINTER(P2PPlan), C.c_void_p,
+                                              C.c_void_p, C.c_size_t, C.c_void_p]),
+    "hedit_unet_workspace_bytes_prepared": (C.c_size_t, [C.c_void_p, C.c_int, C.c_int, C.c_int]),
     "hedit_unet_set_attn_hook": (C.c_int, [C.c_void_p, C.c_void_p, C.c_void_p]),
     "hedit_unet_num_store_layers": (C.c_int, [C.c_void_p, C.c_int, C.c_int]),
     "hedit_unet_store_layer_info": (C.c_int, [C.c_void_p, C.c_int, C.c_int, C.c_int, C.POINTER(C.c_int),
@@ -248,6 +261,9 @@
     "hedit_k_ffn_chain": (C.c_int, [C.c_void_p, C.c_int64, C.c_void_p, C.c_int64, C.c_void_p, C.c_int64, C.c_void_p, C.c_void_p, C.c_void_p,
                                     C.c_float, C.c_void_p, C.c_void_p, C.c_void_p, C.c_void_p, C.c_void_p, C.c_int64, C.c_int, C.c_int,
                                     C.c_void_p]),
+    "hedit_k_ffn_chain_mapped": (C.c_int, [C.c_void_p, C.c_int64, C.c_void_p, C.c_int64, C.c_void_p, C.c_int64, C.c_void_p, C.c_void_p,
+                                           C.c_void_p, C.c_float, C.c_void_p, C.c_void_p, C.c_void_p, C.c_void_p, C.c_void_p, C.c_int64,
+                                           C.c_int, C.c_int, C.POINTER(C.c_int), C.c_int, C.c_int, C.c_int, C.c_void_p]),
     "hedit_k_ffn_fused": (C.c_int, [C.c_void_p, C.c_int64, C.c_void_p, C.c_void_p, C.c_float, C.c_void_p, C.c_void_p,
                                     C.c_void_p, C.c_void_p, C.c_int64, C.c_int, C.c_int, C.c_void_p]),
     "hedit_k_groupnorm_ws_bytes": (C.c_size_t, [C.c_int, C.c_int, C.c_int]),
diff --git a/h-edit_amd/hedit/engine.py b/h-edit_amd/hedit/engine.py
--- a/h-edit_amd/hedit/engine.py
+++ b/h-edit_amd/hedit/engine.py
@@ -53,6 +53,22 @@
         c.coeff = _f(self.edit_coeff(t, t_prev, eta, ddim_inv)) if coeff is None else _f(coeff)
         c.w_rec = float(w_rec)
         return c
+
+
+class _RunContexts:
+
+    def __init__(self, unet, **tensors):
+        self._unet, self._raw, self._prepared = unet, tensors, {}
+
+    def raw(self, name):
+        return self._raw[name]
+
+    def __getattr__(self, name):
+        if name.startswith("_") or name not in self._raw:
+            raise AttributeError(name)
+        if name not in self._prepared:
+            self._prepared[name] = self._unet.prepare_context(self._raw[name])
+        return self._prepared[name]
 
 
 class HEditEngine:
@@ -153,11 +169,10 @@
         else:
             null, src, tar = (c.to(device=dev, dtype=torch.float32) for c in ctx)
         nulln = null.expand(n, -1, -1) if null.shape[0] == 1 else null
-        ctx_base4 = torch.cat([nulln, nulln, src, src]).contiguous()
-        ctx_base2 = torch.cat([nulln, src]).contiguous()
-        ctx_edit = torch.cat([nulln, nulln, src, tar]).contiguous()
-        ctx_src = src.contiguous()
-        ctx_edit5 = torch.cat([nulln, nulln, src, tar, src]).contiguous() if fuse_src_pass else None
+        cx = _RunContexts(self.unet, base4=torch.cat([nulln, nulln, src, src]).contiguous(),
+                          base2=torch.cat([nulln, src]).contiguous(), edit=torch.cat([nulln, nulln, src, tar]).contiguous(),
+                          src=src.contiguous(),
+                          **({"edit5": torch.cat([nulln, nulln, src, tar, src]).contiguous()} if fuse_src_pass else {}))
 
         ts = [int(v) for v in sch.timesteps]
         op = ts[-after_skip_steps:]
@@ -189,9 +204,9 @@
         def p2p_pass(parts, blocks, t, save):
             rows = len(blocks) * n
             if foreign:
-                return self.unet.forward_hooked(torch.cat([parts[b] for b in blocks]), t, ctx_edit, controller, save)
+                return self.unet.forward_hooked(torch.cat([parts[b] for b in blocks]), t, cx.raw("edit"), controller, save)
             plan = controller._plan(self.unet, rows, xT.shape[2], xT.shape[3], save) if controller is not None else None
-            e = unet_rows(parts, blocks, t, ctx_edit5 if rows == 5 * n else ctx_edit, plan)
+            e = unet_rows(parts, blocks, t, cx.edit5 if rows == 5 * n else cx.edit, plan)
             if controller is not None:
                 controller._after_pass(save)
             return e
@@ -207,32 +222,32 @@
 
             if (not p2p) and implicit and i == 0 and ahead != -1:
                 xe = xt[n:]
-                e = unet_rows([xe], (0, 0, 0, 0), t, ctx_edit, off)
+                e = unet_rows([xe], (0, 0, 0, 0), t, cx.edit, off)
                 c0 = S.step_coef(t, tt, eta_i, ddim_inv, cfg_scales, w_rec, coeff=S.edit_coeff(ahead, t, eta_i, ddim_inv))
                 new = torch.empty_like(xe)
                 self.step_update(e[0:n], e[2 * n:3 * n], e[n:2 * n], e[3 * n:], xe, xe, new, n, False, c0)
                 xt = torch.cat([xt[:n], new]).contiguous()
 
             if p2p and reuse and carry is not None:
-                e2 = unet_rows([xt[n:]], (0, 0), t, ctx_base2, off)
+                e2 = unet_rows([xt[n:]], (0, 0), t, cx.base2, off)
                 e = torch.cat([carry[0], e2[:n], carry[1], e2[n:]])
                 self.step_base(e, xt, z, x_prev, n, 4, coef)
             elif p2p:
-                e = unet_rows([xt[:n], xt[n:]], (0, 1, 0, 1), t, ctx_base4, off)
+                e = unet_rows([xt[:n], xt[n:]], (0, 1, 0, 1), t, cx.base4, off)
                 self.step_base(e, xt, z, x_prev, n, 4, coef)
             else:
-                e = unet_rows([xt[n:]], (0, 0), t, ctx_base2, off)
+                e = unet_rows([xt[n:]], (0, 0), t, cx.base2, off)
                 self.step_base(e, xt, z, x_prev, n, 2, coef)
             x_orig, x_base = x_prev[:n], x_prev[n:]
 
             if not implicit:
                 new = torch.empty_like(x_base)
                 if p2p:
-                    e_src = self.unet.forward_raw(xt[n:].contiguous(), t, ctx_src, off)
+                    e_src = self.unet.forward_raw(xt[n:].contiguous(), t, cx.src, off)
                     e = p2p_pass([xt[:n], xt[n:]], (0, 1, 0, 1), t, True)
                     self.step_update(e[n:2 * n], e_src, e[n:2 * n], e[3 * n:], x_base, x_base, new, n, False, coef)
                 else:
-                    e = unet_rows([xt[n:]], (0, 0, 0, 0), t, ctx_edit, off)
+                    e = unet_rows([xt[n:]], (0, 0, 0, 0), t, cx.edit, off)
                     self.step_update(e[0:n], e[2 * n:3 * n], e[n:2 * n], e[3 * n:], x_base, x_base, new, n, False, coef)
                 x_k = new
             else:
@@ -245,7 +260,7 @@
                             e = p2p_pass([x_orig, x_k], (0, 1, 0, 1, 1), tt, save)
                             e_src = e[4 * n:]
                         else:
-                            e_src = self.unet.forward_raw(x_k, tt, ctx_src, off)
+                            e_src = self.unet.forward_raw(x_k, tt, cx.src, off)
                             e = p2p_pass([x_orig, x_k], (0, 1, 0, 1), tt, save)
                         self.step_update(e[n:2 * n], e_src, e[n:2 * n], e[3 * n:4 * n], x_k, x_base, new, n,
                                          k > 0 and style is None and rec_pull, coef)
@@ -256,7 +271,7 @@
                         if reuse:
                             carry = (e[0:n], e[2 * n:3 * n])
                     else:
-                        e = unet_rows([x_k], (0, 0, 0, 0), tt, ctx_edit, off)
+                        e = unet_rows([x_k], (0, 0, 0, 0), tt, cx.edit, off)
                         self.step_update(e[0:n], e[2 * n:3 * n], e[n:2 * n], e[3 * n:], x_k, x_base, new, n, k > 0, coef)
                     x_k = new
 
@@ -285,9 +300,8 @@
                 zs = zs[:, None]
         null = self.encode([""]).expand(n, -1, -1)
         src, tar = self.encode([p[0] for p in pairs]), self.encode([p[1] for p in pairs])
-        ctx_base4 = torch.cat([null, null, src, src]).contiguous()
-        ctx_k2 = torch.cat([null, src]).contiguous()
-        ctx_pair = torch.cat([src, tar]).contiguous()
+        cx = _RunContexts(self.unet, base4=torch.cat([null, null, src, src]).contiguous(),
+                          k2=torch.cat([null, src]).contiguous(), pair=torch.cat([src, tar]).contiguous())
         editor = getattr(self.unet, "_attention_editor", None)
         ts = [int(v) for v in sch.timesteps]
         op = ts[-after_skip_steps:]
@@ -301,15 +315,15 @@
             eta_i = float(eta[idx]) if isinstance(eta, (list, tuple)) else float(eta)
             coef = S.step_coef(t, tt, eta_i, ddim_inv, cfg_scales, 0.0)
             register_time(self.model, t)
-            e = self.unet.forward_raw(torch.cat([xt, xt]), t, ctx_base4, None)
+            e = self.unet.forward_raw(torch.cat([xt, xt]), t, cx.base4, None)
             self.step_base(e, xt, z, x_prev, n, 4, coef)
             x_orig, x_base = x_prev[:n], x_prev[n:]
             x_k = x_base.clone()
             for _ in range(K):
                 register_time(self.model, tt)
-                e2 = self.unet.forward_raw(torch.cat([x_k, x_k]), tt, ctx_k2, None)
+                e2 = self.unet.forward_raw(torch.cat([x_k, x_k]), tt, cx.k2, None)
                 plan = editor._plan(self.unet, 2 * n, H, W, True, n_images=n) if editor is not None else None
-                ep = self.unet.forward_raw(torch.cat([x_orig, x_k]), tt, ctx_pair, plan)
+                ep = self.unet.forward_raw(torch.cat([x_orig, x_k]), tt, cx.pair, plan)
                 if editor is not None:
                     editor._after_pass(True)
                 new = torch.empty_like(x_k)
@@ -356,6 +370,7 @@
         else:
             ctx = torch.cat([null, tar]).contiguous()
         controlled = control and kinds == 2 and controller is not None
+        cx = _RunContexts(self.unet, rows=ctx)
 
         from .p2p.ptp_classes import runs_in_python
         foreign = controlled and runs_in_python(controller)
@@ -380,10 +395,10 @@
             if foreign:
                 e = self.unet.forward_hooked(x_in, t, ctx, controller, True)
             elif controlled:
-                e = self.unet.forward_raw(x_in, t, ctx, controller._plan(self.unet, 4 * n, H, W, True))
+                e = self.unet.forward_raw(x_in, t, cx.rows, controller._plan(self.unet, 4 * n, H, W, True))
                 controller._after_pass(True)
             else:
-                e = self.unet.forward_raw(x_in, t, ctx, None)
+                e = self.unet.forward_raw(x_in, t, cx.rows, None)
             coefs = self._pair_coefs(S, t, eta_i, ddim_inv, cfg_pair)
             x_next = torch.empty_like(xt)
             self.step_pair(e[:kinds * n], e[kinds * n:], xt, z, x_next, n, kinds, coefs[:kinds])
@@ -418,8 +433,7 @@
                 zs = zs[:, None]
         src, tar = self.encode([p[0] for p in pairs]), self.encode([p[1] for p in pairs])
         u = src if uncond == "src" else self.encode([""]).expand(n, -1, -1)
-        ctx_u = torch.cat([u, u]).contiguous()
-        ctx_pair = torch.cat([src, tar]).contiguous()
+        cx = _RunContexts(self.unet, u=torch.cat([u, u]).contiguous(), pair=torch.cat([src, tar]).contiguous())
         editor = getattr(self.unet, "_attention_editor", None)
         ts = [int(v) for v in sch.timesteps]
         op = ts[-after_skip_steps:]
@@ -430,9 +444,9 @@
             z = zs[idx] if zs is not None else None
             eta_i = float(eta[idx]) if isinstance(eta, (list, tuple)) else float(eta)
             register_time(self.model, t)
-            e_u = self.unet.forward_raw(xt, t, ctx_u, None)
+            e_u = self.unet.forward_raw(xt, t, cx.u, None)
             plan = editor._plan(self.unet, 2 * n, H, W, True, n_images=n) if editor is not None else None
-            e_c = self.unet.forward_raw(xt, t, ctx_pair, plan)
+            e_c = self.unet.forward_raw(xt, t, cx.pair, plan)
             if editor is not None:
                 editor._after_pass(True)
             x_next = torch.empty_like(xt)
@@ -466,6 +480,7 @@
         null = self.encode([""]).expand(n, -1, -1)
         cond = any(p != "" for p in prompts)
         ctx = torch.cat([null, self.encode(list(prompts))]).contiguous() if cond else null.contiguous()
+        ctx = self.unet.prepare_context(ctx)
         zs = torch.zeros(T, *x0.shape, device=dev)
         for i, t in enumerate(ts):
             idx = T - i - 1
diff --git a/h-edit_amd/hedit/unet.py b/h-edit_amd/hedit/unet.py
--- a/h-edit_amd/hedit/unet.py
+++ b/h-edit_amd/hedit/unet.py
@@ -31,6 +31,16 @@
 
 class AttnProcessor:
     controller = None
+
+
+class PreparedContext:
+
+    def __init__(self, ctx, buf, desc):
+        self.ctx, self.buf, self.desc = ctx, buf, desc
+
+    @property
+    def shape(self):
+        return self.ctx.shape
 
 
 def random_state_dict(param_shapes, seed=0):
@@ -227,10 +237,31 @@
         _lib.check(self._lib.hedit_prof_records(self._h, rows.ctypes.data_as(C.POINTER(C.c_double)), max_rows, C.byref(n)))
         return rows[:n.value]
 
+    def prepare_context(self, ctx):
+        if ctx.dtype != torch.float32 or ctx.dim() != 3 or ctx.shape[1:] != (77, self.config["cross_attention_dim"]):
+            raise ValueError(f"encoder_hidden_states must be float32 (B, 77, {self.config['cross_attention_dim']}), "
+                             f"got {ctx.dtype} {tuple(ctx.shape)}")
+        ctx = ctx.to(self.device).contiguous()
+        B = ctx.shape[0]
+        with torch.cuda.device(self.device):
+            buf = torch.empty(self._lib.hedit_unet_context_bytes(self._h, B), dtype=torch.uint8, device=self.device)
+            need = self._lib.hedit_unet_context_workspace_bytes(self._h, B)
+            if self._ws is None or self._ws.numel() < need:
+                self._ws = None
+                self._ws = torch.empty(need, dtype=torch.uint8, device=self.device)
+            desc = _lib.UnetContext()
+            _lib.check(self._lib.hedit_unet_context_prepare(self._h, _lib.ptr(ctx), B, _lib.ptr(buf), buf.numel(),
+                                                            _lib.ptr(self._ws), self._ws.numel(), _lib.cur_stream(),
+                                                            C.byref(desc)))
+        return PreparedContext(ctx, buf, desc)
+
     def forward_raw(self, sample, t, ctx, plan=None, out=None, row_latent=None):
         B, Cc, H, W = sample.shape
         if row_latent is not None:
             B = len(row_latent)
+        prepared = None
+        if isinstance(ctx, PreparedContext):
+            prepared, ctx = ctx, ctx.ctx
         if sample.dtype != torch.float32 or ctx.dtype != torch.float32:
             raise TypeError("sample and encoder_hidden_states must be float32")
         if ctx.shape != (B, 77, self.config["cross_attention_dim"]):
@@ -241,16 +272,11 @@
         if out is None:
             out = torch.empty(B, self.config["out_channels"], H, W, dtype=torch.float32, device=sample.device)
         ws = self._workspace(B, H, W)
-        if row_latent is None:
-            _lib.check(self._lib.hedit_unet_forward(
-                self._h, _lib.ptr(sample), C.c_float(float(t)), _lib.ptr(ctx), B, H, W,
-                C.byref(plan) if plan is not None else None, _lib.ptr(out), _lib.ptr(ws), ws.numel(),
-                _lib.cur_stream()))
-            return out
-        if sample.data_ptr() % 16:
+        if row_latent is not None and sample.data_ptr() % 16:
             sample = sample.clone()
-        _lib.check(self._lib.hedit_unet_forward_shared(
-            self._h, _lib.ptr(sample), sample.shape[0], (C.c_int * B)(*row_latent), C.c_float(float(t)), _lib.ptr(ctx), B, H, W,
+        _lib.check(self._lib.hedit_unet_forward_prepared(
+            self._h, _lib.ptr(sample), sample.shape[0], (C.c_int * B)(*row_latent) if row_latent is not None else None,
+            C.c_float(float(t)), _lib.ptr(ctx), C.byref(prepared.desc) if prepared is not None else None, B, H, W,
             C.byref(plan) if plan is not None else None, _lib.ptr(out), _lib.ptr(ws), ws.numel(),
             _lib.cur_stream()))
         return out
@@ -278,6 +304,8 @@
         _lib.check(self._lib.hedit_unet_set_attn_hook(self._h, C.cast(fn, C.c_void_p), None))
         try:
             try:
+                if isinstance(ctx, PreparedContext):
+                    ctx = ctx.ctx
                 return self.forward_raw(sample, t, ctx, None, out)
             except _lib.HipError:
                 if state["exc"] is not None:
diff --git a/include/hedit.h b/include/hedit.h
--- a/include/hedit.h
+++ b/include/hedit.h
@@ -67,6 +67,20 @@
 int hedit_unet_forward_shared(hedit_unet* h, const float* x, int D, const int* row_latent, float t, const float* ctx, int B,
                               int height, int width, const hedit_p2p_plan* plan, float* eps_out, void* workspace,
                               size_t workspace_bytes, void* stream);
+typedef struct hedit_unet_context {
+  void* buf;
+  size_t bytes;
+  int B, ctx_n, storage_f16, reserved;
+  uint64_t epoch;
+} hedit_unet_context;
+size_t hedit_unet_context_bytes(const hedit_unet* h, int B);
+size_t hedit_unet_context_workspace_bytes(hedit_unet* h, int B);
+int hedit_unet_context_prepare(hedit_unet* h, const float* ctx, int B, void* buf, size_t buf_bytes, void* workspace,
+                               size_t workspace_bytes, void* stream, hedit_unet_context* out);
+int hedit_unet_forward_prepared(hedit_unet* h, const float* x, int D, const int* row_latent, float t, const float* ctx,
+                                const hedit_unet_context* prepared, int B, int height, int width, const hedit_p2p_plan* plan,
+                                float* eps_out, void* workspace, size_t workspace_bytes, void* stream);
+size_t hedit_unet_workspace_bytes_prepared(hedit_unet* h, int B, int height, int width);
 typedef int (*hedit_attn_hook_fn)(void* user, float* probs, int batch_heads, int n_query, int n_key, int is_cross, int place,
                                   int layer, void* stream);
 int hedit_unet_set_attn_hook(hedit_unet* h, hedit_attn_hook_fn fn, void* user);
@@ -157,6 +171,10 @@
 int hedit_k_ffn_chain(const void* a, int64_t lda, const void* t1, int64_t ldt1, const void* x, int64_t ldx, const float* bias_pre,
                       const float* gamma, const float* beta, float eps, const void* w_stream, const float* bias1_packed,
                       const float* bias2, const float* bias_post, void* out, int64_t ldo, int M, int C, void* stream);
+int hedit_k_ffn_chain_mapped(const void* a, int64_t lda, const void* t1, int64_t ldt1, const void* x, int64_t ldx,
+                             const float* bias_pre, const float* gamma, const float* beta, float eps, const void* w_stream,
+                             const float* bias1_packed, const float* bias2, const float* bias_post, void* out, int64_t ldo, int M,
+                             int C, const int* image_map, int n_images, int src_images, int rows_per_image, void* stream);
 size_t hedit_k_lin_chain_stream_bytes(int n_out);
 int hedit_k_lin_chain_pack(const float* w_pre, const float* w0, const float* w1, const float* w2, float scale0, void* stream_out,
                            void* stream);
```

After: 2.606, median of 6. No clear change (+0.7%).
